# apple/swift-homomorphic-encryption

Hardware: NVIDIA H100
Metric: BFV ct*ct mults/sec at N=8192, 4 coefficient moduli (higher is better)
Workload: dtype u64

## Files before the change

swift-homomorphic-encryption_b200/csrc/behz.cu:

```cuda
#include <cstdlib>

#include "kernels.cuh"
#include "ntt_fast.cuh"

namespace hecuda {

constexpr int kThreads = 128;

static int cols_per_thread() {
    static const int v = [] {
        const char *e = std::getenv("HECUDA_BEHZ_COLS");
        return (e && e[0] == '1') ? 1 : 2;
    }();
    return v;
}

template <int COLS>
struct Cols {
    u64 v[COLS];
};
template <int COLS>
__device__ __forceinline__ Cols<COLS> ldc(const u64 *p) {
    Cols<COLS> r;
    if (COLS == 2) {
        const ulonglong2 t = *reinterpret_cast<const ulonglong2 *>(p);
        r.v[0] = t.x;
        r.v[COLS - 1] = t.y;
    } else {
        r.v[0] = *p;
    }
    return r;
}
template <int COLS>
__device__ __forceinline__ void stc(u64 *p, const u64 (&v)[COLS]) {
    if (COLS == 2) *reinterpret_cast<ulonglong2 *>(p) = make_ulonglong2(v[0], v[COLS - 1]);
    else *p = v[0];
}

template <int L, int COLS, bool H>
__global__ void __launch_bounds__(kThreads) lift_kernel(const u64 *__restrict__ in, int polys_in, u64 *__restrict__ ext,
                                                       int ext_polys, int out_poly_offset,
                                                       const __grid_constant__ LiftConsts c, int n, bool q_rows) {
    const int rows_out = q_rows ? 2 * L + 1 : L + 1, aux0 = q_rows ? L : 0;
    const int coeff = (blockIdx.x * kThreads + threadIdx.x) * COLS;
    if (coeff >= n) return;
    const int64_t poly = (int64_t)blockIdx.z * gridDim.y + blockIdx.y;
    const int64_t item = polys_in == 2 ? (poly >> 1) : poly / polys_in;
    const int pin = (int)(poly - item * polys_in);
    const u64 *src = in + poly * L * n + coeff;
    u64 *dst = ext + ((item * ext_polys + out_poly_offset + pin) * rows_out) * n + coeff;
    u64 z[COLS][L];
    u32 acc_mt[COLS];
#pragma unroll
    for (int k = 0; k < COLS; ++k) acc_mt[k] = 0;
#pragma unroll
    for (int i = 0; i < L; ++i) {
        const Cols<COLS> x = ldc<COLS>(src + (int64_t)i * n);
        if (q_rows) stc<COLS>(dst + (int64_t)i * n, x.v);
#pragma unroll
        for (int k = 0; k < COLS; ++k) {
            z[k][i] = shoup_mul(x.v[k], c.in_w[i], c.in_wp[i], c.q[i]);
            acc_mt[k] += (u32)z[k][i] * c.punct_mt[i];
        }
    }
    u32 r[COLS];
    bool neg[COLS];
#pragma unroll
    for (int k = 0; k < COLS; ++k) {
        r[k] = (acc_mt[k] * c.neg_inv_q_mt) & c.mt_mask;
        neg[k] = r[k] >= c.mt_half;
    }
#pragma unroll
    for (int j = 0; j <= L; ++j) {
        u64 o[COLS];
#pragma unroll
        for (int k = 0; k < COLS; ++k) {
            const u64 rc = neg[k] ? (u64)r[k] + c.neg_off[j] : (u64)r[k];
            u128 acc = (u128)rc * c.qr[j];
#pragma unroll
            for (int i = 0; i < L; ++i) mac128(acc, z[k][i], c.mat[j][i]);
            const u64 red = mont_reduce_c<H>(acc, c.b[j], c.b_ninv[j]);
            o[k] = c.wide_sums ? barrett64(red, c.b[j], c.b_mu1[j]) : csub(red, c.b[j]);
        }
        stc<COLS>(dst + (int64_t)(aux0 + j) * n, o);
    }
}

struct TensorConsts {
    int R;
    u64 p[kMaxRows], ninv[kMaxRows];
    unsigned char h[kMaxRows];
};

template <int COLS, bool H>
__device__ __forceinline__ void tensor_cols(const Cols<COLS> &a0, const Cols<COLS> &a1, const Cols<COLS> &b0,
                                            const Cols<COLS> &b1, u64 p, u64 ninv, u64 (&o0)[COLS], u64 (&o1)[COLS],
                                            u64 (&o2)[COLS]) {
#pragma unroll
    for (int k = 0; k < COLS; ++k) {
        o0[k] = csub(mont_reduce_c<H>((u128)a0.v[k] * b0.v[k], p, ninv), p);
        u128 m = (u128)a0.v[k] * b1.v[k];
        mac128(m, a1.v[k], b0.v[k]);
        o1[k] = csub(mont_reduce_c<H>(m, p, ninv), p);
        o2[k] = csub(mont_reduce_c<H>((u128)a1.v[k] * b1.v[k], p, ninv), p);
    }
}

template <int COLS, bool ANY_H>
__global__ void __launch_bounds__(kThreads) tensor_kernel(const u64 *__restrict__ ext, u64 *__restrict__ ten,
                                                         const __grid_constant__ TensorConsts c, int n) {
    const int R = c.R;
    const int row = blockIdx.y;
    const int64_t item = blockIdx.z;
    const int coeff = (blockIdx.x * kThreads + threadIdx.x) * COLS;
    if (coeff >= n) return;
    const u64 p = c.p[row], ninv = c.ninv[row];
    const u64 *e = ext + (item * 4 * R + row) * n + coeff;
    const int64_t ps = (int64_t)R * n;
    const Cols<COLS> a0 = ldc<COLS>(e), a1 = ldc<COLS>(e + ps), b0 = ldc<COLS>(e + 2 * ps), b1 = ldc<COLS>(e + 3 * ps);
    u64 *o = ten + (item * 3 * R + row) * n + coeff;
    u64 o0[COLS], o1[COLS], o2[COLS];
    if (ANY_H && c.h[row]) tensor_cols<COLS, true>(a0, a1, b0, b1, p, ninv, o0, o1, o2);
    else tensor_cols<COLS, false>(a0, a1, b0, b1, p, ninv, o0, o1, o2);
    stc<COLS>(o, o0);
    stc<COLS>(o + ps, o1);
    stc<COLS>(o + 2 * ps, o2);
}

struct TensorSumConsts {
    int R;
    long long max_pairs;
    u64 p[kMaxRows], ninv[kMaxRows], mu1[kMaxRows], mu_hi[kMaxRows], mu_lo[kMaxRows];
};

__global__ void __launch_bounds__(kThreads) tensor_sum_kernel(const u64 *__restrict__ ext, u64 *__restrict__ ten,
                                                             const __grid_constant__ TensorSumConsts c, int n,
                                                             long long pairs) {
    const int R = c.R;
    const int row = blockIdx.y;
    const int64_t group = blockIdx.z;
    const int coeff = (blockIdx.x * kThreads + threadIdx.x) * 2;
    if (coeff >= n) return;
    const u64 p = c.p[row], ninv = c.ninv[row];
    const int64_t ps = (int64_t)R * n;
    const u64 *e = ext + (group * pairs * 4 * R + row) * n + coeff;
    u128 a0[2] = {0, 0}, a1[2] = {0, 0}, a2[2] = {0, 0};
    long long since = 0;
    for (long long k = 0; k < pairs; ++k, e += 4 * ps) {
        const Cols<2> l0 = ldc<2>(e), l1 = ldc<2>(e + ps), r0 = ldc<2>(e + 2 * ps), r1 = ldc<2>(e + 3 * ps);
#pragma unroll
        for (int j = 0; j < 2; ++j) {
            mac128(a0[j], l0.v[j], r0.v[j]);
            mac128(a1[j], l0.v[j], r1.v[j]);
            mac128(a1[j], l1.v[j], r0.v[j]);
            mac128(a2[j], l1.v[j], r1.v[j]);
        }
        if (++since >= c.max_pairs) {
            since = 0;
#pragma unroll
            for (int j = 0; j < 2; ++j) {
                u128w w0 = {(u64)a0[j], (u64)(a0[j] >> 64)}, w1 = {(u64)a1[j], (u64)(a1[j] >> 64)},
                      w2 = {(u64)a2[j], (u64)(a2[j] >> 64)};
                a0[j] = barrett128(w0, p, c.mu_hi[row], c.mu_lo[row]);
                a1[j] = barrett128(w1, p, c.mu_hi[row], c.mu_lo[row]);
                a2[j] = barrett128(w2, p, c.mu_hi[row], c.mu_lo[row]);
            }
        }
    }
    u64 *o = ten + (group * 3 * R + row) * n + coeff;
    u64 o0[2], o1[2], o2[2];
    const u64 mu1 = c.mu1[row];
#pragma unroll
    for (int j = 0; j < 2; ++j) {
        o0[j] = barrett64(mont_reduce(a0[j], p, ninv), p, mu1);
        o1[j] = barrett64(mont_reduce(a1[j], p, ninv), p, mu1);
        o2[j] = barrett64(mont_reduce(a2[j], p, ninv), p, mu1);
    }
    stc<2>(o, o0);
    stc<2>(o + ps, o1);
    stc<2>(o + 2 * ps, o2);
}

template <int L, int COLS, bool H>
__global__ void __launch_bounds__(kThreads) floor_kernel(const u64 *__restrict__ in, u64 *__restrict__ out,
                                                        const __grid_constant__ FloorConsts c, int n) {
    constexpr int R = 2 * L + 1;
    const int coeff = (blockIdx.x * kThreads + threadIdx.x) * COLS;
    if (coeff >= n) return;
    const int64_t poly = (int64_t)blockIdx.z * gridDim.y + blockIdx.y;
    const u64 *src = in + poly * R * n + coeff;
    u64 *dst = out + poly * L * n + coeff;
    u64 y[COLS][L];
#pragma unroll
    for (int i = 0; i < L; ++i) {
        const Cols<COLS> x = ldc<COLS>(src + (int64_t)i * n);
#pragma unroll
        for (int k = 0; k < COLS; ++k) y[k][i] = shoup_mul(x.v[k], c.inq_w[i], c.inq_wp[i], c.q[i]);
    }
    u64 f[COLS][L + 1];
#pragma unroll
    for (int j = 0; j <= L; ++j) {
        const Cols<COLS> xb = ldc<COLS>(src + (int64_t)(L + j) * n);
#pragma unroll
        for (int k = 0; k < COLS; ++k) {
            u128 acc = (u128)xb.v[k] * c.fq[j];
#pragma unroll
            for (int i = 0; i < L; ++i) mac128(acc, y[k][i], c.fmat[j][i]);
            f[k][j] = mont_reduce_c<H>(acc, c.b[j], c.b_ninv[j]);
        }
    }
    const u64 msk = c.b[L];
    u64 outv[L][COLS];
#pragma unroll
    for (int k = 0; k < COLS; ++k) {
        u64 w[L];
        u128 acc = (u128)f[k][L] * c.a_msk;
#pragma unroll
        for (int i = 0; i < L; ++i) {
            w[i] = shoup_mul(f[k][i], c.inb_w[i], c.inb_wp[i], c.b[i]);
            mac128(acc, w[i], c.amat[i]);
        }
        u64 alpha = mont_reduce_c<H>(acc, msk, c.b_ninv[L]);
        alpha = c.wide_sums ? barrett64(alpha, msk, c.msk_mu1) : csub(csub(csub(alpha, 4 * msk), 2 * msk), msk);
        const bool exceeds = alpha > (msk >> 1);
        const u64 alpha_c = exceeds ? msk - alpha : alpha;
#pragma unroll
        for (int i = 0; i < L; ++i) {
            u128 o = (u128)alpha_c * (exceeds ? c.b_mod_q[i] : c.neg_b_mod_q[i]);
#pragma unroll
            for (int kk = 0; kk < L; ++kk) mac128(o, w[kk], c.omat[i][kk]);
            outv[i][k] = csub(csub(mont_reduce(o, c.q[i], c.q_ninv[i]), 2 * c.q[i]), c.q[i]);
        }
    }
#pragma unroll
    for (int i = 0; i < L; ++i) stc<COLS>(dst + (int64_t)i * n, outv[i]);
}

__global__ void __launch_bounds__(kThreads) lift_generic_kernel(const u64 *__restrict__ in, int polys_in, u64 *__restrict__ ext,
                                                               int ext_polys, int out_poly_offset,
                                                               const __grid_constant__ LiftConsts c, int n, bool q_rows) {
    const int L = c.L, rows_out = q_rows ? 2 * L + 1 : L + 1, aux0 = q_rows ? L : 0;
    const int coeff = blockIdx.x * kThreads + threadIdx.x;
    if (coeff >= n) return;
    const int64_t poly = (int64_t)blockIdx.z * gridDim.y + blockIdx.y;
    const int64_t item = poly / polys_in;
    const int pin = (int)(poly - item * polys_in);
    const u64 *src = in + poly * L * n + coeff;
    u64 *dst = ext + ((item * ext_polys + out_poly_offset + pin) * rows_out) * n + coeff;
    u64 z[kMaxL];
    u32 acc_mt = 0;
    for (int i = 0; i < L; ++i) {
        const u64 x = src[(int64_t)i * n];
        if (q_rows) dst[(int64_t)i * n] = x;
        z[i] = shoup_mul(x, c.in_w[i], c.in_wp[i], c.q[i]);
        acc_mt += (u32)z[i] * c.punct_mt[i];
    }
    const u32 r = (acc_mt * c.neg_inv_q_mt) & c.mt_mask;
    const bool neg = r >= c.mt_half;
    for (int j = 0; j <= L; ++j) {
        const u64 rc = neg ? (u64)r + c.neg_off[j] : (u64)r;
        u128 acc = (u128)rc * c.qr[j];
        for (int i = 0; i < L; ++i) mac128(acc, z[i], c.mat[j][i]);
        const u64 red = mont_reduce(acc, c.b[j], c.b_ninv[j]);
        dst[(int64_t)(aux0 + j) * n] = c.wide_sums ? barrett64(red, c.b[j], c.b_mu1[j]) : csub(red, c.b[j]);
    }
}

__global__ void __launch_bounds__(kThreads) floor_generic_kernel(const u64 *__restrict__ in, u64 *__restrict__ out,
                                                                const __grid_constant__ FloorConsts c, int n) {
    const int L = c.L, R = 2 * L + 1;
    const int coeff = blockIdx.x * kThreads + threadIdx.x;
    if (coeff >= n) return;
    const int64_t poly = (int64_t)blockIdx.z * gridDim.y + blockIdx.y;
    const u64 *src = in + poly * R * n + coeff;
    u64 *dst = out + poly * L * n + coeff;
    u64 y[kMaxL], f[kMaxL + 1], w[kMaxL];
    for (int i = 0; i < L; ++i) y[i] = shoup_mul(src[(int64_t)i * n], c.inq_w[i], c.inq_wp[i], c.q[i]);
    for (int j = 0; j <= L; ++j) {
        u128 acc = (u128)src[(int64_t)(L + j) * n] * c.fq[j];
        for (int i = 0; i < L; ++i) mac128(acc, y[i], c.fmat[j][i]);
        f[j] = mont_reduce(acc, c.b[j], c.b_ninv[j]);
    }
    const u64 msk = c.b[L];
    u128 acc = (u128)f[L] * c.a_msk;
    for (int i = 0; i < L; ++i) {
        w[i] = shoup_mul(f[i], c.inb_w[i], c.inb_wp[i], c.b[i]);
        mac128(acc, w[i], c.amat[i]);
    }
    u64 alpha = mont_reduce(acc, msk, c.b_ninv[L]);
    alpha = c.wide_sums ? barrett64(alpha, msk, c.msk_mu1) : csub(csub(csub(alpha, 4 * msk), 2 * msk), msk);
    const bool exceeds = alpha > (msk >> 1);
    const u64 alpha_c = exceeds ? msk - alpha : alpha;
    for (int i = 0; i < L; ++i) {
        u128 o = (u128)alpha_c * (exceeds ? c.b_mod_q[i] : c.neg_b_mod_q[i]);
        for (int kk = 0; kk < L; ++kk) mac128(o, w[kk], c.omat[i][kk]);
        dst[(int64_t)i * n] = barrett64(mont_reduce(o, c.q[i], c.q_ninv[i]), c.q[i], c.q_mu1[i]);
    }
}

#define HE_DISPATCH_L(L_, CALL)                                                                                       \
    switch (L_) {                                                                                                     \
        case 1: { constexpr int LL = 1; CALL; } break;                                                                \
        case 2: { constexpr int LL = 2; CALL; } break;                                                                \
        case 3: { constexpr int LL = 3; CALL; } break;                                                                \
        case 4: { constexpr int LL = 4; CALL; } break;                                                                \
        case 5: { constexpr int LL = 5; CALL; } break;                                                                \
        case 6: { constexpr int LL = 6; CALL; } break;                                                                \
        case 7: { constexpr int LL = 7; CALL; } break;                                                                \
        case 8: { constexpr int LL = 8; CALL; } break;                                                                \
        case 9: { constexpr int LL = 9; CALL; } break;                                                                \
        case 10: { constexpr int LL = 10; CALL; } break;                                                              \
        case 11: { constexpr int LL = 11; CALL; } break;                                                              \
        case 12: { constexpr int LL = 12; CALL; } break;                                                              \
        case 13: { constexpr int LL = 13; CALL; } break;                                                              \
        case 14: { constexpr int LL = 14; CALL; } break;                                                              \
        case 15: { constexpr int LL = 15; CALL; } break;                                                              \
        case 16: { constexpr int LL = 16; CALL; } break;                                                              \
        default: return cudaErrorInvalidValue;                                                                        \
    }

template <int COLS, bool H>
static cudaError_t launch_lift_kernel(int L, dim3 grid, cudaStream_t stream, const u64 *in, int polys_in, u64 *ext,
                                      int ext_polys, int out_poly_offset, const LiftConsts &consts, int n, bool q_rows) {
    HE_DISPATCH_L(L, (lift_kernel<LL, COLS, H><<<grid, kThreads, 0, stream>>>(in, polys_in, ext, ext_polys, out_poly_offset,
                                                                              consts, n, q_rows)));
    return cudaSuccess;
}
template <int COLS, bool H>
static cudaError_t launch_floor_kernel(int L, dim3 grid, cudaStream_t stream, const u64 *in, u64 *out,
                                       const FloorConsts &consts, int n) {
    HE_DISPATCH_L(L, (floor_kernel<LL, COLS, H><<<grid, kThreads, 0, stream>>>(in, out, consts, n)));
    return cudaSuccess;
}

static inline dim3 poly_grid(int64_t n, int64_t polys, int cols) {
    const unsigned gx = (unsigned)((n / cols + kThreads - 1) / kThreads);
    const int64_t gy = polys < 32768 ? polys : 32768;
    return dim3(gx ? gx : 1, (unsigned)gy, (unsigned)((polys + gy - 1) / gy));
}

cudaError_t launch_lift(const Context &ctx, const u64 *in, int polys_in, u64 *ext, int ext_polys, int out_poly_offset,
                        int64_t items, cudaStream_t stream, bool reference_base, bool q_rows) {
    const LiftConsts &consts = reference_base ? ctx.lift : ctx.lift_mul;
    int64_t polys = items * polys_in;
    if (polys == 0) return cudaSuccess;
    const int64_t pstride_in = (int64_t)ctx.L * ctx.n;
    while (polys > 0) {
        int64_t slab = polys >= 32768 ? (polys / 32768) * 32768 : polys;
        const int cols = ctx.L > 16 ? 1 : (ctx.n >= 2 ? cols_per_thread() : 1);
        const dim3 grid = poly_grid(ctx.n, slab, cols);
        ++g_kernel_launches;
        if (ctx.L > 16) {
            lift_generic_kernel<<<grid, kThreads, 0, stream>>>(in, polys_in, ext, ext_polys, out_poly_offset, consts, (int)ctx.n, q_rows);
        } else {
            auto launch = cols == 2 ? (consts.h_primes ? launch_lift_kernel<2, true> : launch_lift_kernel<2, false>)
                                    : (consts.h_primes ? launch_lift_kernel<1, true> : launch_lift_kernel<1, false>);
            const cudaError_t e = launch(ctx.L, grid, stream, in, polys_in, ext, ext_polys, out_poly_offset, consts, (int)ctx.n, q_rows);
            if (e != cudaSuccess) return e;
        }
        in += slab * pstride_in;
        ext += (slab / polys_in) * (int64_t)ext_polys * (q_rows ? 2 * ctx.L + 1 : ctx.L + 1) * ctx.n;
        polys -= slab;
    }
    return cudaGetLastError();
}

cudaError_t launch_tensor(const Context &ctx, const u64 *ext, u64 *ten, int64_t items, cudaStream_t stream,
                          bool reference_base) {
    if (items == 0) return cudaSuccess;
    TensorConsts tc;
    tc.R = 2 * ctx.L + 1;
    const NttRowMap map = reference_base ? ctx.map_qbsk() : ctx.map_qaux();
    for (int r = 0; r < tc.R; ++r) {
        tc.p[r] = ctx.slots[map.slot[r]].dev.p;
        tc.ninv[r] = ctx.slots[map.slot[r]].dev.ninv;
        tc.h[r] = fast::class_of_modulus(tc.p[r], ctx.slots[map.slot[r]].dev.bits) == fast::kNarrowH ? 1 : 0;
    }
    const int cols = ctx.n >= 2 ? cols_per_thread() : 1;
    bool any_h = false;
    for (int r = 0; r < tc.R; ++r) any_h |= tc.h[r] != 0;
    auto k = cols == 2 ? (any_h ? tensor_kernel<2, true> : tensor_kernel<2, false>) : (any_h ? tensor_kernel<1, true> : tensor_kernel<1, false>);
    const unsigned gx = (unsigned)((ctx.n / cols + kThreads - 1) / kThreads);
    for (int64_t done = 0; done < items;) {
        const int64_t chunk = (items - done) > 65535 ? 65535 : (items - done);
        dim3 grid(gx ? gx : 1, (unsigned)tc.R, (unsigned)chunk);
        ++g_kernel_launches;
        k<<<grid, kThreads, 0, stream>>>(ext + done * 4 * tc.R * ctx.n, ten + done * 3 * tc.R * ctx.n, tc, (int)ctx.n);
        done += chunk;
    }
    return cudaGetLastError();
}

cudaError_t launch_tensor_sum(const Context &ctx, const u64 *ext, u64 *ten, int64_t pairs, int64_t groups,
                              cudaStream_t stream, bool reference_base) {
    if (groups == 0) return cudaSuccess;
    if (ctx.n < 2 || pairs < 1) return cudaErrorInvalidValue;
    TensorSumConsts tc;
    tc.R = 2 * ctx.L + 1;
    const NttRowMap map = reference_base ? ctx.map_qbsk() : ctx.map_qaux();
    u64 pmax = 0;
    for (int r = 0; r < tc.R; ++r) {
        const ModSlot &S = ctx.slots[map.slot[r]].dev;
        tc.p[r] = S.p;
        tc.ninv[r] = S.ninv;
        tc.mu1[r] = S.mu1;
        tc.mu_hi[r] = S.mu_hi;
        tc.mu_lo[r] = S.mu_lo;
        pmax = S.p > pmax ? S.p : pmax;
    }
    const u128 per_pair = 2 * (u128)pmax * pmax;
    const u128 cap = (((u128)1) << 127) / per_pair;
    tc.max_pairs = cap < 1 ? 1 : (cap > (u128)0x7fffffffLL ? 0x7fffffffLL : (long long)cap);
    const unsigned gx = (unsigned)((ctx.n / 2 + kThreads - 1) / kThreads);
    for (int64_t done = 0; done < groups;) {
        const int64_t chunk = (groups - done) > 65535 ? 65535 : (groups - done);
        dim3 grid(gx ? gx : 1, (unsigned)tc.R, (unsigned)chunk);
        ++g_kernel_launches;
        tensor_sum_kernel<<<grid, kThreads, 0, stream>>>(ext + done * pairs * 4 * tc.R * ctx.n, ten + done * 3 * tc.R * ctx.n,
                                                         tc, (int)ctx.n, pairs);
        done += chunk;
    }
    return cudaGetLastError();
}

cudaError_t launch_floor(const Context &ctx, const u64 *in, u64 *out, int64_t polys, cudaStream_t stream,
                         bool reference_base) {
    if (polys == 0) return cudaSuccess;
    const FloorConsts &consts = reference_base ? ctx.floor : ctx.floor_mul;
    const int R = 2 * ctx.L + 1;
    while (polys > 0) {
        int64_t slab = polys >= 32768 ? (polys / 32768) * 32768 : polys;
        const int cols = ctx.L > 16 ? 1 : (ctx.n >= 2 ? cols_per_thread() : 1);
        const dim3 grid = poly_grid(ctx.n, slab, cols);
        ++g_kernel_launches;
        if (ctx.L > 16) {
            floor_generic_kernel<<<grid, kThreads, 0, stream>>>(in, out, consts, (int)ctx.n);
        } else {
            auto launch = cols == 2 ? (consts.h_primes ? launch_floor_kernel<2, true> : launch_floor_kernel<2, false>)
                                    : (consts.h_primes ? launch_floor_kernel<1, true> : launch_floor_kernel<1, false>);
            const cudaError_t e = launch(ctx.L, grid, stream, in, out, consts, (int)ctx.n);
            if (e != cudaSuccess) return e;
        }
        in += slab * (int64_t)R * ctx.n;
        out += slab * (int64_t)ctx.L * ctx.n;
        polys -= slab;
    }
    return cudaGetLastError();
}

}
```

swift-homomorphic-encryption_b200/csrc/capi.cu:

```cuda
#include "../../include/hecuda.h"

#include <cuda_runtime.h>
#include <sched.h>
#include <sys/syscall.h>
#include <unistd.h>

#include <algorithm>
#include <cctype>
#include <cstdio>
#include <cstdlib>
#include <cstring>
#include <map>
#include <memory>
#include <mutex>
#include <new>
#include <string>
#include <vector>

#include "capi_internal.hpp"

namespace hecuda {
std::atomic<unsigned long long> g_kernel_launches{0};
}

using namespace hecuda;

namespace hecuda {
namespace api {

static thread_local std::string tl_error;

int32_t fail(int32_t code, const std::string &msg) {
    tl_error = msg;
    return code;
}
int32_t cuda_fail(cudaError_t e, const char *what) {
    return fail(HECUDA_ERR_CUDA, std::string(what) + ": " + cudaGetErrorString(e));
}
const char *last_error_cstr() { return tl_error.c_str(); }

}
}

using namespace hecuda::api;

namespace hecuda {
namespace api {

cudaError_t wait_stream(cudaStream_t s) {
    static const bool blocking = [] {
        const char *env = std::getenv("HECUDA_BLOCKING_SYNC");
        return !(env && env[0] == '0');
    }();
    if (!blocking) return cudaStreamSynchronize(s);
    thread_local cudaEvent_t event = nullptr;
    thread_local int event_device = -1;
    int device = 0;
    cudaError_t e = cudaGetDevice(&device);
    if (e != cudaSuccess) return e;
    if (!event || event_device != device) {
        if ((e = cudaEventCreateWithFlags(&event, cudaEventBlockingSync | cudaEventDisableTiming)) != cudaSuccess) return e;
        event_device = device;
    }
    if ((e = cudaEventRecord(event, s)) != cudaSuccess) return e;
    return cudaEventSynchronize(event);
}

int32_t check_ctx(const hecuda_context *h) {
    if (!h || !h->ctx) return fail(HECUDA_ERR_INVALID_ARGUMENT, "invalidContext: null context");
    int dev = -1;
    if (cudaGetDevice(&dev) != cudaSuccess) return fail(HECUDA_ERR_NO_DEVICE, "no CUDA device available");
    if (dev != h->ctx->device) {
        cudaError_t e = cudaSetDevice(h->ctx->device);
        if (e != cudaSuccess) return cuda_fail(e, "cudaSetDevice");
    }
    return HECUDA_OK;
}

bool make_map(const Context &c, int32_t base, int32_t rows, NttRowMap &map, std::string &err) {
    switch (base) {
        case HECUDA_BASE_Q:
            if (rows < 1 || rows > c.L) { err = "invalidPolyContext: row_count must be in [1, L] for BASE_Q"; return false; }
            map = c.map_q(rows);
            return true;
        case HECUDA_BASE_Q_BSK:
            if (rows != 2 * c.L + 1) { err = "invalidPolyContext: BASE_Q_BSK needs 2L+1 rows"; return false; }
            map = c.map_qbsk();
            return true;
        case HECUDA_BASE_Q_AUX:
            if (rows != 2 * c.L + 1) { err = "invalidPolyContext: BASE_Q_AUX needs 2L+1 rows"; return false; }
            map = c.map_qaux();
            return true;
        case HECUDA_BASE_KEYSWITCH:
            if (!c.has_ks) { err = "invalidPolyContext: these parameters have no key-switching modulus"; return false; }
            if (rows < 2 || rows > c.L + 1) { err = "invalidPolyContext: BASE_KEYSWITCH needs 2..L+1 rows"; return false; }
            map = c.map_ks(rows - 1);
            return true;
        default:
            err = "invalidPolyContext: unknown base";
            return false;
    }
}


size_t multiply_scratch_words(const Context &c) { return (size_t)7 * (2 * c.L + 1) * c.n; }
size_t relinearize_scratch_words(const Context &c, int l) { return (size_t)((l + 1) * l + 2 * (l + 1)) * c.n; }

cudaError_t multiply_chunk(const Context &c, u64 *scratch, const u64 *lhs, const u64 *rhs, u64 *out, int64_t items,
                           cudaStream_t s) {
    const int R = 2 * c.L + 1;
    const size_t poly_words = (size_t)R * c.n;
    cudaError_t e;
    u64 *ext = scratch, *ten = scratch + 4 * poly_words * items;
    const NttRowMap map = c.map_qaux();
    if (ntt_forward_tensor_supported(c)) {
        if ((e = launch_lift(c, lhs, 2, ext, 4, 0, items, s, false, false)) != cudaSuccess) return e;
        if ((e = launch_lift(c, rhs, 2, ext, 4, 2, items, s, false, false)) != cudaSuccess) return e;
        if ((e = launch_ntt_forward_tensor(c, map, lhs, rhs, ext, ten, items, s)) != cudaSuccess) return e;
        if ((e = launch_ntt_inverse(c, map, ten, ten, items * 3 * R, kScaleTMont, s)) != cudaSuccess) return e;
        return launch_floor(c, ten, out, items * 3, s);
    }
    if ((e = launch_lift(c, lhs, 2, ext, 4, 0, items, s)) != cudaSuccess) return e;
    if ((e = launch_lift(c, rhs, 2, ext, 4, 2, items, s)) != cudaSuccess) return e;
    if ((e = launch_ntt_forward(c, map, ext, ext, items * 4 * R, s)) != cudaSuccess) return e;
    if ((e = launch_tensor(c, ext, ten, items, s)) != cudaSuccess) return e;
    if ((e = launch_ntt_inverse(c, map, ten, ten, items * 3 * R, kScaleTMont, s)) != cudaSuccess) return e;
    return launch_floor(c, ten, out, items * 3, s);
}

cudaError_t keyswitch_chunk(const Context &c, u64 *scratch, const u64 *key, const u64 *target, int64_t target_stride,
                            int l, const u64 *base, int64_t base_stride, int base_mask, u64 *out, int64_t items,
                            cudaStream_t s) {
    const size_t dig_words = (size_t)(l + 1) * l * c.n;
    cudaError_t e;
    u64 *dig = scratch, *prod = scratch + dig_words * items;
    if ((e = launch_ntt_forward(c, c.map_ks_digits(l, target_stride), target, dig, items * (l + 1) * l, s)) != cudaSuccess)
        return e;
    if ((e = launch_ks_mac(c, dig, key, l, prod, items, s)) != cudaSuccess) return e;
    if ((e = launch_ntt_inverse(c, c.map_ks(l), prod, prod, items * 2 * (l + 1), kScaleMont, s)) != cudaSuccess) return e;
    return launch_ks_finish(c, prod, base, base_stride, base_mask, l, out, items, s);
}

cudaError_t relinearize_chunk(const Context &c, u64 *scratch, const u64 *key, const u64 *ct3, int l, u64 *out,
                              int64_t items, cudaStream_t s) {
    const int64_t ct_stride = (int64_t)3 * l * c.n;
    return keyswitch_chunk(c, scratch, key, ct3 + (int64_t)2 * l * c.n, ct_stride, l, ct3, ct_stride, 3, out, items, s);
}

size_t galois_scratch_words(const Context &c, int l) { return relinearize_scratch_words(c, l) + (size_t)l * c.n; }
cudaError_t apply_galois_chunk(const Context &c, u64 *scratch, const u64 *key, const u64 *ct, int l, unsigned element,
                               u64 *out, int64_t items, cudaStream_t s) {
    const int64_t poly = (int64_t)l * c.n, ct_stride = 2 * poly;
    u64 *perm1 = scratch;
    u64 *ks_scratch = scratch + poly * items;
    const NttRowMap map = c.map_q(l);
    cudaError_t e;
    if ((e = launch_galois_coeff(c, map, element, ct, ct_stride, out, ct_stride, items, s)) != cudaSuccess) return e;
    if ((e = launch_galois_coeff(c, map, element, ct + poly, ct_stride, perm1, poly, items, s)) != cudaSuccess) return e;
    return keyswitch_chunk(c, ks_scratch, key, perm1, poly, l, out, ct_stride, 1, out, items, s);
}

cudaError_t inner_product_chunk(const Context &c, u64 *scratch, const u64 *lhs, const u64 *rhs, int64_t pairs,
                                       u64 *out, int64_t groups, cudaStream_t s) {
    const int R = 2 * c.L + 1;
    const size_t poly_words = (size_t)R * c.n;
    const int64_t items = groups * pairs;
    u64 *ext = scratch, *ten = scratch + 4 * poly_words * items;
    const NttRowMap map = c.map_qaux();
    cudaError_t e;
    if ((e = launch_lift(c, lhs, 2, ext, 4, 0, items, s)) != cudaSuccess) return e;
    if ((e = launch_lift(c, rhs, 2, ext, 4, 2, items, s)) != cudaSuccess) return e;
    if ((e = launch_ntt_forward(c, map, ext, ext, items * 4 * R, s)) != cudaSuccess) return e;
    if ((e = launch_tensor_sum(c, ext, ten, pairs, groups, s)) != cudaSuccess) return e;
    if ((e = launch_ntt_inverse(c, map, ten, ten, groups * 3 * R, kScaleTMont, s)) != cudaSuccess) return e;
    return launch_floor(c, ten, out, groups * 3, s);
}
size_t inner_product_scratch_words(const Context &c, int64_t pairs) {
    return (size_t)(4 * pairs + 3) * (2 * c.L + 1) * c.n;
}

}
}

namespace {

thread_local bool tl_io32 = false;
struct Io32Scope {
    Io32Scope() { tl_io32 = true; }
    ~Io32Scope() { tl_io32 = false; }
};

struct HostIo {
    const u64 *src;
    size_t words_per_item;
};
template <class Body>
int32_t host_pipeline(const hecuda_context *h, int64_t batch, int64_t chunk_hint, size_t scratch_words_per_item,
                      const std::vector<HostIo> &inputs, u64 *host_out, size_t out_words_per_item, Body body) {
    if (batch == 0) return HECUDA_OK;
    static const int depth = [] {
        const char *env = std::getenv("HECUDA_PIPELINE_DEPTH");
        const int d = env ? std::atoi(env) : 3;
        return d < 1 ? 1 : (d > 8 ? 8 : d);
    }();
    static const int64_t min_stages = [] {
        const char *env = std::getenv("HECUDA_PIPELINE_STAGES");
        const long long v = env ? std::atoll(env) : 16;
        return (int64_t)(v < 1 ? 1 : v);
    }();
    std::vector<std::unique_ptr<WsGuard>> guards;
    std::vector<Workspace *> ws;
    for (int i = 0; i < depth; ++i) {
        guards.emplace_back(new WsGuard(h));
        if (!guards.back()->w) return fail(HECUDA_ERR_CUDA, "could not create a CUDA stream / workspace");
        ws.push_back(guards.back()->w);
    }
    int64_t chunk = std::max<int64_t>(1, std::min<int64_t>(chunk_hint, batch));
    if (batch >= 64) chunk = std::min<int64_t>(chunk, std::max<int64_t>(16, (batch + min_stages - 1) / min_stages));
    struct DrainOnExit {
        std::vector<Workspace *> &ws;
        ~DrainOnExit() {
            for (Workspace *w : ws) wait_stream(w->stream);
        }
    } drain{ws};
    int k = 0;
    for (int64_t done = 0; done < batch; done += chunk, ++k) {
        Workspace &w = *ws[k % depth];
        const int64_t items = std::min<int64_t>(chunk, batch - done);
        size_t in_words = 0;
        for (const HostIo &io : inputs) in_words += io.words_per_item * (size_t)items;
        const bool io32 = tl_io32;
        const size_t out_words = out_words_per_item * (size_t)items;
        CK(w.reserve(0, scratch_words_per_item * (size_t)items));
        CK(w.reserve(4, in_words));
        CK(w.reserve(5, out_words));
        if (io32) {
            CK(w.reserve(6, in_words / 2 + inputs.size() * 2 + 2));
            CK(w.reserve(7, out_words / 2 + 2));
        }
        std::vector<const u64 *> d_in;
        size_t off = 0, off32 = 0;
        for (const HostIo &io : inputs) {
            const size_t words = io.words_per_item * (size_t)items;
            if (io32) {
                u32 *raw = reinterpret_cast<u32 *>(w.buf[6]) + off32;
                CK(cudaMemcpyAsync(raw, reinterpret_cast<const u32 *>(io.src) + io.words_per_item * (size_t)done,
                                   words * sizeof(u32), cudaMemcpyHostToDevice, w.stream));
                CK(launch_widen(raw, w.buf[4] + off, (int64_t)words, w.stream));
                off32 += (words + 3) & ~(size_t)3;
            } else {
                CK(cudaMemcpyAsync(w.buf[4] + off, io.src + io.words_per_item * (size_t)done, words * sizeof(u64),
                                   cudaMemcpyHostToDevice, w.stream));
            }
            d_in.push_back(w.buf[4] + off);
            off += words;
        }
        cudaError_t e = body(w, d_in, w.buf[5], items);
        if (e != cudaSuccess) return cuda_fail(e, "kernel launch");
        if (io32) {
            CK(launch_narrow(w.buf[5], reinterpret_cast<u32 *>(w.buf[7]), (int64_t)out_words, w.stream));
            CK(cudaMemcpyAsync(reinterpret_cast<u32 *>(host_out) + out_words_per_item * (size_t)done, w.buf[7],
                               out_words * sizeof(u32), cudaMemcpyDeviceToHost, w.stream));
        } else {
            CK(cudaMemcpyAsync(host_out + out_words_per_item * (size_t)done, w.buf[5], out_words * sizeof(u64),
                               cudaMemcpyDeviceToHost, w.stream));
        }
    }
    for (Workspace *w : ws) CK(wait_stream(w->stream));
    return HECUDA_OK;
}

}


extern "C" {

int32_t hecuda_version(void) { return 100; }
const char *hecuda_last_error(void) { return last_error_cstr(); }

int32_t hecuda_device_count(int32_t *count) {
    if (!count) return fail(HECUDA_ERR_INVALID_ARGUMENT, "null count");
    int n = 0;
    cudaError_t e = cudaGetDeviceCount(&n);
    if (e != cudaSuccess) {
        *count = 0;
        return fail(HECUDA_ERR_NO_DEVICE, std::string("no CUDA device: ") + cudaGetErrorString(e));
    }
    *count = n;
    return HECUDA_OK;
}
int32_t hecuda_set_device(int32_t device) {
    CK(cudaSetDevice(device));
    return HECUDA_OK;
}

int32_t hecuda_bind_host_to_device(int32_t device, int32_t *numa_node, int32_t *cpu_count) {
    if (numa_node) *numa_node = -1;
    if (cpu_count) *cpu_count = 0;
    char bus[32] = {0};
    CK(cudaDeviceGetPCIBusId(bus, sizeof(bus), device));
    for (char *c = bus; *c; ++c) *c = (char)std::tolower((unsigned char)*c);
    const std::string dir = std::string("/sys/bus/pci/devices/") + bus + "/";
    int node = -1;
    if (FILE *f = std::fopen((dir + "numa_node").c_str(), "r")) {
        if (std::fscanf(f, "%d", &node) != 1) node = -1;
        std::fclose(f);
    }
    char list[4096] = {0};
    if (FILE *f = std::fopen((dir + "local_cpulist").c_str(), "r")) {
        if (!std::fgets(list, sizeof(list), f)) list[0] = 0;
        std::fclose(f);
    }
    cpu_set_t current, want;
    CPU_ZERO(&want);
    if (sched_getaffinity(0, sizeof(current), &current) != 0) return HECUDA_OK;
    int picked = 0;
    char *save = nullptr;
    for (char *tok = strtok_r(list, ",\n", &save); tok; tok = strtok_r(nullptr, ",\n", &save)) {
        int lo = 0, hi = 0;
        const int fields = std::sscanf(tok, "%d-%d", &lo, &hi);
        if (fields < 1) continue;
        if (fields == 1) hi = lo;
        for (int c = lo; c <= hi && c < CPU_SETSIZE; ++c)
            if (CPU_ISSET(c, &current)) {
                CPU_SET(c, &want);
                ++picked;
            }
    }
    if (picked > 0) sched_setaffinity(0, sizeof(want), &want);
    if (node >= 0 && node < 64) {
        unsigned long mask = 1ul << node;
        syscall(SYS_set_mempolicy, 1 , &mask, sizeof(mask) * 8);
    }
    if (numa_node) *numa_node = node;
    if (cpu_count) *cpu_count = picked;
    return HECUDA_OK;
}

int32_t hecuda_host_alloc(void **ptr, uint64_t bytes) {
    if (!ptr) return fail(HECUDA_ERR_INVALID_ARGUMENT, "null ptr");
    CK(cudaHostAlloc(ptr, bytes, cudaHostAllocDefault));
    return HECUDA_OK;
}
int32_t hecuda_host_free(void *ptr) {
    CK(cudaFreeHost(ptr));
    return HECUDA_OK;
}
int32_t hecuda_host_register(void *ptr, uint64_t bytes) {
    CK(cudaHostRegister(ptr, bytes, cudaHostRegisterDefault));
    return HECUDA_OK;
}
int32_t hecuda_host_unregister(void *ptr) {
    CK(cudaHostUnregister(ptr));
    return HECUDA_OK;
}

static int32_t context_create(int64_t poly_degree, const uint64_t *coefficient_moduli, int32_t moduli_count,
                              uint64_t plaintext_modulus, int word_bits, hecuda_context **out);
int32_t hecuda_context_create(int64_t poly_degree, const uint64_t *coefficient_moduli, int32_t moduli_count,
                              uint64_t plaintext_modulus, hecuda_context **out) {
    return context_create(poly_degree, coefficient_moduli, moduli_count, plaintext_modulus, 64, out);
}
int32_t hecuda_context_create_u32(int64_t poly_degree, const uint32_t *coefficient_moduli, int32_t moduli_count,
                                  uint32_t plaintext_modulus, hecuda_context **out) {
    if (!coefficient_moduli || moduli_count < 0) return fail(HECUDA_ERR_INVALID_ARGUMENT, "null argument");
    std::vector<uint64_t> wide(coefficient_moduli, coefficient_moduli + moduli_count);
    return context_create(poly_degree, wide.data(), moduli_count, plaintext_modulus, 32, out);
}
int32_t hecuda_context_word_bits(const hecuda_context *h, int32_t *bits) {
    if (!h || !bits) return fail(HECUDA_ERR_INVALID_ARGUMENT, "null argument");
    *bits = h->ctx->word_bits;
    return HECUDA_OK;
}
static int32_t context_create(int64_t poly_degree, const uint64_t *coefficient_moduli, int32_t moduli_count,
                              uint64_t plaintext_modulus, int word_bits, hecuda_context **out) {
    if (!out || !coefficient_moduli) return fail(HECUDA_ERR_INVALID_ARGUMENT, "null argument");
    *out = nullptr;
    int ndev = 0;
    if (cudaGetDeviceCount(&ndev) != cudaSuccess || ndev == 0)
        return fail(HECUDA_ERR_NO_DEVICE, "no CUDA device: libhecuda has no CPU fallback");
    std::string err;
    Context *c = Context::create(poly_degree, (const u64 *)coefficient_moduli, moduli_count, plaintext_modulus, err, word_bits);
    if (!c) {
        const bool unsupported = err.rfind("unsupported", 0) == 0;
        return fail(unsupported ? HECUDA_ERR_UNSUPPORTED : HECUDA_ERR_INVALID_ARGUMENT, err);
    }
    hecuda_context *h = new (std::nothrow) hecuda_context();
    if (!h) {
        delete c;
        return fail(HECUDA_ERR_CUDA, "out of host memory");
    }
    h->ctx = c;
    {
        cudaMemPool_t pool;
        if (cudaDeviceGetDefaultMemPool(&pool, c->device) == cudaSuccess) {
            unsigned long long threshold = ~0ull;
            cudaMemPoolSetAttribute(pool, cudaMemPoolAttrReleaseThreshold, &threshold);
        }
    }
    const size_t per_item = (size_t)7 * (2 * c->L + 1) * c->n * sizeof(u64);
    int64_t chunk = (int64_t)((size_t)2048 * 1024 * 1024 / per_item);
    if (const char *env = std::getenv("HECUDA_CHUNK")) chunk = std::atoll(env);
    h->chunk = std::max<int64_t>(1, std::min<int64_t>(chunk, 4096));
    context_registered(h, true);
    *out = h;
    return HECUDA_OK;
}

int32_t hecuda_context_destroy(hecuda_context *h) {
    if (!h) return HECUDA_OK;
    if (h->ctx) cudaSetDevice(h->ctx->device);
    cudaDeviceSynchronize();
    pir_graphs_purge(h, nullptr);
    context_registered(h, false);
    for (Workspace *w : h->free_ws) {
        w->release();
        delete w;
    }
    delete h->ctx;
    delete h;
    return HECUDA_OK;
}

int32_t hecuda_context_ciphertext_moduli_count(const hecuda_context *h, int32_t *count) {
    if (!h || !count) return fail(HECUDA_ERR_INVALID_ARGUMENT, "null argument");
    *count = h->ctx->L;
    return HECUDA_OK;
}
int32_t hecuda_context_bsk_moduli(const hecuda_context *h, uint64_t *out, int32_t capacity, int32_t *count) {
    if (!h || !count) return fail(HECUDA_ERR_INVALID_ARGUMENT, "null argument");
    *count = (int32_t)h->ctx->bsk.size();
    if (out) {
        if (capacity < *count) return fail(HECUDA_ERR_INVALID_ARGUMENT, "capacity too small");
        std::memcpy(out, h->ctx->bsk.data(), sizeof(u64) * h->ctx->bsk.size());
    }
    return HECUDA_OK;
}
int32_t hecuda_context_aux_moduli(const hecuda_context *h, uint64_t *out, int32_t capacity, int32_t *count) {
    if (!h || !count) return fail(HECUDA_ERR_INVALID_ARGUMENT, "null argument");
    *count = (int32_t)h->ctx->aux.size();
    if (out) {
        if (capacity < *count) return fail(HECUDA_ERR_INVALID_ARGUMENT, "capacity too small");
        std::memcpy(out, h->ctx->aux.data(), sizeof(u64) * h->ctx->aux.size());
    }
    return HECUDA_OK;
}
int32_t hecuda_context_root_tables(const hecuda_context *h, uint64_t modulus, uint64_t *roots, uint64_t *inverse_roots) {
    if (!h) return fail(HECUDA_ERR_INVALID_ARGUMENT, "null context");
    const int s = h->ctx->find_slot(modulus);
    if (s < 0) return fail(HECUDA_ERR_INVALID_ARGUMENT, "invalidNttModulus: modulus is not part of this context");
    if (roots) std::memcpy(roots, h->ctx->slots[s].roots.data(), sizeof(u64) * h->ctx->n);
    if (inverse_roots) std::memcpy(inverse_roots, h->ctx->slots[s].inv_roots.data(), sizeof(u64) * h->ctx->n);
    return HECUDA_OK;
}


static int32_t ntt_device(const hecuda_context *h, int32_t base, uint64_t *data, int32_t rows, int64_t polys,
                          void *stream, bool inverse) {
    int32_t rc = check_ctx(h);
    if (rc) return rc;
    if (polys < 0 || (!data && polys)) return fail(HECUDA_ERR_INVALID_ARGUMENT, "invalid data / poly_count");
    NttRowMap map;
    std::string err;
    if (!make_map(*h->ctx, base, rows, map, err)) return fail(HECUDA_ERR_INVALID_ARGUMENT, err);
    cudaError_t e = inverse ? launch_ntt_inverse(*h->ctx, map, (u64 *)data, (u64 *)data, polys * rows, kScalePlain,
                                                 (cudaStream_t)stream)
                            : launch_ntt_forward(*h->ctx, map, (u64 *)data, (u64 *)data, polys * rows,
                                                 (cudaStream_t)stream);
    if (e != cudaSuccess) return cuda_fail(e, "ntt launch");
    return HECUDA_OK;
}
int32_t hecuda_ntt_forward_device(const hecuda_context *h, int32_t base, uint64_t *data, int32_t rows, int64_t polys,
                                  void *stream) {
    return ntt_device(h, base, data, rows, polys, stream, false);
}
int32_t hecuda_ntt_inverse_device(const hecuda_context *h, int32_t base, uint64_t *data, int32_t rows, int64_t polys,
                                  void *stream) {
    return ntt_device(h, base, data, rows, polys, stream, true);
}

static int32_t ntt_host(const hecuda_context *h, const NttRowMap &map, uint64_t *data, size_t words_per_item,
                        int64_t items, int64_t rows_per_item, bool inverse) {
    const Context &c = *h->ctx;
    std::vector<HostIo> in = {{(const u64 *)data, words_per_item}};
    const int64_t chunk = std::max<int64_t>(1, (int64_t)((size_t)4 * 1024 * 1024 / std::max<size_t>(1, words_per_item)));
    return host_pipeline(h, items, chunk, 0, in, (u64 *)data, words_per_item,
                         [&](Workspace &w, const std::vector<const u64 *> &d_in, u64 *d_out, int64_t n_items) {
                             return inverse ? launch_ntt_inverse(c, map, d_in[0], d_out, n_items * rows_per_item, kScalePlain,
                                                                 w.stream)
                                            : launch_ntt_forward(c, map, d_in[0], d_out, n_items * rows_per_item,
                                                                 w.stream);
                         });
}
int32_t hecuda_ntt_forward(const hecuda_context *h, int32_t base, uint64_t *data, int32_t rows, int64_t polys) {
    int32_t rc = check_ctx(h);
    if (rc) return rc;
    if (polys < 0 || (!data && polys)) return fail(HECUDA_ERR_INVALID_ARGUMENT, "invalid data / poly_count");
    NttRowMap map;
    std::string err;
    if (!make_map(*h->ctx, base, rows, map, err)) return fail(HECUDA_ERR_INVALID_ARGUMENT, err);
    return ntt_host(h, map, data, (size_t)rows * h->ctx->n, polys, rows, false);
}
int32_t hecuda_ntt_inverse(const hecuda_context *h, int32_t base, uint64_t *data, int32_t rows, int64_t polys) {
    int32_t rc = check_ctx(h);
    if (rc) return rc;
    if (polys < 0 || (!data && polys)) return fail(HECUDA_ERR_INVALID_ARGUMENT, "invalid data / poly_count");
    NttRowMap map;
    std::string err;
    if (!make_map(*h->ctx, base, rows, map, err)) return fail(HECUDA_ERR_INVALID_ARGUMENT, err);
    return ntt_host(h, map, data, (size_t)rows * h->ctx->n, polys, rows, true);
}
int32_t hecuda_rnstool_lift_q_to_qbsk(const hecuda_context *h, const uint64_t *polys, uint64_t *out, int64_t count) {
    int32_t rc = check_ctx(h);
    if (rc) return rc;
    if (count < 0 || ((!polys || !out) && count)) return fail(HECUDA_ERR_INVALID_ARGUMENT, "invalid buffers / poly_count");
    const Context &c = *h->ctx;
    const size_t in_words = (size_t)c.L * c.n, out_words = (size_t)(2 * c.L + 1) * c.n;
    std::vector<HostIo> in = {{(const u64 *)polys, in_words}};
    return host_pipeline(h, count, std::max<int64_t>(1, (int64_t)((size_t)4 * 1024 * 1024 / out_words)), 0, in, (u64 *)out, out_words,
                         [&](Workspace &w, const std::vector<const u64 *> &d_in, u64 *d_out, int64_t n_items) {
                             return launch_lift(c, d_in[0], 1, d_out, 1, 0, n_items, w.stream, true);
                         });
}
int32_t hecuda_rnstool_floor_qbsk_to_q(const hecuda_context *h, const uint64_t *polys, uint64_t *out, int64_t count) {
    int32_t rc = check_ctx(h);
    if (rc) return rc;
    if (count < 0 || ((!polys || !out) && count)) return fail(HECUDA_ERR_INVALID_ARGUMENT, "invalid buffers / poly_count");
    const Context &c = *h->ctx;
    const size_t in_words = (size_t)(2 * c.L + 1) * c.n, out_words = (size_t)c.L * c.n;
    std::vector<HostIo> in = {{(const u64 *)polys, in_words}};
    return host_pipeline(h, count, std::max<int64_t>(1, (int64_t)((size_t)4 * 1024 * 1024 / in_words)), 0, in, (u64 *)out, out_words,
                         [&](Workspace &w, const std::vector<const u64 *> &d_in, u64 *d_out, int64_t n_items) {
                             return launch_floor(c, d_in[0], d_out, n_items, w.stream, true);
                         });
}

static int32_t ntt_rows_host(const hecuda_context *h, uint64_t modulus, uint64_t *data, int64_t rows, bool inverse) {
    int32_t rc = check_ctx(h);
    if (rc) return rc;
    if (rows < 0 || (!data && rows)) return fail(HECUDA_ERR_INVALID_ARGUMENT, "invalid data / row_count");
    const int s = h->ctx->find_slot(modulus);
    if (s < 0) return fail(HECUDA_ERR_INVALID_ARGUMENT, "invalidPolyContext: modulus is not part of this context");
    return ntt_host(h, h->ctx->map_single(s), data, (size_t)h->ctx->n, rows, 1, inverse);
}
int32_t hecuda_ntt_forward_rows(const hecuda_context *h, uint64_t modulus, uint64_t *data, int64_t rows) {
    return ntt_rows_host(h, modulus, data, rows, false);
}
int32_t hecuda_ntt_inverse_rows(const hecuda_context *h, uint64_t modulus, uint64_t *data, int64_t rows) {
    return ntt_rows_host(h, modulus, data, rows, true);
}


int32_t hecuda_bfv_multiply_device(const hecuda_context *h, const uint64_t *lhs, const uint64_t *rhs, uint64_t *out,
                                   int64_t batch, void *stream) {
    int32_t rc = check_ctx(h);
    if (rc) return rc;
    if (batch < 0 || (batch && (!lhs || !rhs || !out))) return fail(HECUDA_ERR_INVALID_ARGUMENT, "invalidCiphertext: null buffer");
    if (batch == 0) return HECUDA_OK;
    const Context &c = *h->ctx;
    const size_t in_words = (size_t)2 * c.L * c.n, out_words = (size_t)3 * c.L * c.n;
    const int64_t chunk = std::max<int64_t>(1, std::min<int64_t>(h->chunk, batch));
    cudaStream_t s = (cudaStream_t)stream;
    u64 *scratch = nullptr;
    CK(cudaMallocAsync(&scratch, multiply_scratch_words(c) * (size_t)chunk * sizeof(u64), s));
    for (int64_t done = 0; done < batch; done += chunk) {
        const int64_t items = std::min<int64_t>(chunk, batch - done);
        cudaError_t e = multiply_chunk(c, scratch, (const u64 *)lhs + in_words * done, (const u64 *)rhs + in_words * done,
                                       (u64 *)out + out_words * done, items, s);
        if (e != cudaSuccess) {
            cudaFreeAsync(scratch, s);
            return cuda_fail(e, "multiply");
        }
    }
    CK(cudaFreeAsync(scratch, s));
    return HECUDA_OK;
}

int32_t hecuda_bfv_multiply(const hecuda_context *h, const uint64_t *lhs, const uint64_t *rhs, uint64_t *out,
                            int64_t batch) {
    int32_t rc = check_ctx(h);
    if (rc) return rc;
    if (batch < 0 || (batch && (!lhs || !rhs || !out))) return fail(HECUDA_ERR_INVALID_ARGUMENT, "invalidCiphertext: null buffer");
    const Context &c = *h->ctx;
    const size_t in_words = (size_t)2 * c.L * c.n, out_words = (size_t)3 * c.L * c.n;
    std::vector<HostIo> in = {{(const u64 *)lhs, in_words}, {(const u64 *)rhs, in_words}};
    return host_pipeline(h, batch, h->chunk, multiply_scratch_words(c), in, (u64 *)out, out_words,
                         [&](Workspace &w, const std::vector<const u64 *> &d_in, u64 *d_out, int64_t items) {
                             return multiply_chunk(c, w.buf[0], d_in[0], d_in[1], d_out, items, w.stream);
                         });
}


int32_t hecuda_evk_create_empty(const hecuda_context *h, hecuda_evk **out) {
    int32_t rc = check_ctx(h);
    if (rc) return rc;
    if (!out) return fail(HECUDA_ERR_INVALID_ARGUMENT, "null argument");
    const Context &c = *h->ctx;
    if (!c.has_ks)
        return fail(HECUDA_ERR_UNSUPPORTED, "unsupportedHeOperation: a single coefficient modulus leaves no key-switching modulus");
    hecuda_evk *k = new (std::nothrow) hecuda_evk();
    if (!k) return fail(HECUDA_ERR_CUDA, "out of host memory");
    k->owner = h;
    k->words = (size_t)c.L * 2 * (c.L + 1) * c.n;
    cudaError_t e = cudaMalloc(&k->d_relin, k->words * sizeof(u64));
    if (e != cudaSuccess) {
        delete k;
        return cuda_fail(e, "cudaMalloc(evk)");
    }
    *out = k;
    return HECUDA_OK;
}
int32_t hecuda_evk_create(const hecuda_context *h, const uint64_t *relin_key, hecuda_evk **out) {
    if (!relin_key) return fail(HECUDA_ERR_MISSING_KEY, "missingRelinearizationKey");
    int32_t rc = hecuda_evk_create_empty(h, out);
    if (rc) return rc;
    cudaError_t e = upload((*out)->d_relin, relin_key, (*out)->words * sizeof(u64));
    if (e != cudaSuccess) {
        hecuda_evk_destroy(*out);
        *out = nullptr;
        return cuda_fail(e, "cudaMemcpy(evk)");
    }
    (*out)->loaded = true;
    return HECUDA_OK;
}
int32_t hecuda_evk_destroy(hecuda_evk *k) {
    if (!k) return HECUDA_OK;
    if (k->owner) pir_graphs_purge(const_cast<hecuda_context *>(k->owner), k);
    if (k->d_relin) cudaFree(k->d_relin);
    for (auto &kv : k->galois) cudaFree(kv.second);
    for (hecuda::u64 *p : k->retired) cudaFree(p);
    delete k;
    return HECUDA_OK;
}
int32_t hecuda_evk_device_buffer(hecuda_evk *k, void **device_ptr, uint64_t *bytes) {
    if (!k || !device_ptr || !bytes) return fail(HECUDA_ERR_INVALID_ARGUMENT, "null argument");
    *device_ptr = k->d_relin;
    *bytes = k->words * sizeof(u64);
    k->loaded = true;
    ++k->version;
    return HECUDA_OK;
}


static int32_t check_relin(const hecuda_context *h, const hecuda_evk *k, const uint64_t *ct3, int32_t l, uint64_t *out,
                           int64_t batch) {
    int32_t rc = check_ctx(h);
    if (rc) return rc;
    if (!k || !k->loaded) return fail(HECUDA_ERR_MISSING_KEY, "missingRelinearizationKey");
    if (k->owner != h) return fail(HECUDA_ERR_INVALID_ARGUMENT, "invalidContext: evaluation key belongs to another context");
    if (l < 1 || l > h->ctx->L) return fail(HECUDA_ERR_INVALID_ARGUMENT, "invalidCiphertext: moduli_count out of range");
    if (batch < 0 || (batch && (!ct3 || !out))) return fail(HECUDA_ERR_INVALID_ARGUMENT, "invalidCiphertext: null buffer");
    return HECUDA_OK;
}

int32_t hecuda_bfv_relinearize_device(const hecuda_context *h, const hecuda_evk *k, const uint64_t *ct3, int32_t l,
                                      uint64_t *out, int64_t batch, void *stream) {
    int32_t rc = check_relin(h, k, ct3, l, out, batch);
    if (rc) return rc;
    if (batch == 0) return HECUDA_OK;
    const Context &c = *h->ctx;
    const size_t in_words = (size_t)3 * l * c.n, out_words = (size_t)2 * l * c.n;
    const int64_t chunk = std::max<int64_t>(1, std::min<int64_t>(h->chunk, batch));
    cudaStream_t s = (cudaStream_t)stream;
    u64 *scratch = nullptr;
    CK(cudaMallocAsync(&scratch, relinearize_scratch_words(c, l) * (size_t)chunk * sizeof(u64), s));
    for (int64_t done = 0; done < batch; done += chunk) {
        const int64_t items = std::min<int64_t>(chunk, batch - done);
        cudaError_t e = relinearize_chunk(c, scratch, k->d_relin, (const u64 *)ct3 + in_words * done, l,
                                          (u64 *)out + out_words * done, items, s);
        if (e != cudaSuccess) {
            cudaFreeAsync(scratch, s);
            return cuda_fail(e, "relinearize");
        }
    }
    CK(cudaFreeAsync(scratch, s));
    return HECUDA_OK;
}

int32_t hecuda_bfv_relinearize(const hecuda_context *h, const hecuda_evk *k, const uint64_t *ct3, int32_t l,
                               uint64_t *out, int64_t batch) {
    int32_t rc = check_relin(h, k, ct3, l, out, batch);
    if (rc) return rc;
    const Context &c = *h->ctx;
    std::vector<HostIo> in = {{(const u64 *)ct3, (size_t)3 * l * c.n}};
    return host_pipeline(h, batch, h->chunk, relinearize_scratch_words(c, l), in, (u64 *)out, (size_t)2 * l * c.n,
                         [&](Workspace &w, const std::vector<const u64 *> &d_in, u64 *d_out, int64_t items) {
                             return relinearize_chunk(c, w.buf[0], k->d_relin, d_in[0], l, d_out, items, w.stream);
                         });
}

static int32_t check_ms(const hecuda_context *h, const uint64_t *ct, int32_t polys, int32_t l, uint64_t *out,
                        int64_t batch) {
    int32_t rc = check_ctx(h);
    if (rc) return rc;
    if (polys < 1) return fail(HECUDA_ERR_INVALID_ARGUMENT, "invalidCiphertext: poly_count");
    if (l < 2 || l > h->ctx->L)
        return fail(HECUDA_ERR_INVALID_ARGUMENT, "invalidPolyContext: modSwitchDown needs a next context (2 <= moduli_count <= L)");
    if (batch < 0 || (batch && (!ct || !out))) return fail(HECUDA_ERR_INVALID_ARGUMENT, "invalidCiphertext: null buffer");
    return HECUDA_OK;
}

int32_t hecuda_bfv_mod_switch_down_device(const hecuda_context *h, const uint64_t *ct, int32_t polys, int32_t l,
                                          uint64_t *out, int64_t batch, void *stream) {
    int32_t rc = check_ms(h, ct, polys, l, out, batch);
    if (rc) return rc;
    cudaError_t e = launch_mod_switch(*h->ctx, (const u64 *)ct, l, (u64 *)out, batch * polys, (cudaStream_t)stream);
    if (e != cudaSuccess) return cuda_fail(e, "mod_switch");
    return HECUDA_OK;
}

int32_t hecuda_bfv_mod_switch_down(const hecuda_context *h, const uint64_t *ct, int32_t polys, int32_t l, uint64_t *out,
                                   int64_t batch) {
    int32_t rc = check_ms(h, ct, polys, l, out, batch);
    if (rc) return rc;
    const Context &c = *h->ctx;
    std::vector<HostIo> in = {{(const u64 *)ct, (size_t)polys * l * c.n}};
    const int64_t chunk = std::max<int64_t>(1, (int64_t)((size_t)4 * 1024 * 1024 / ((size_t)polys * l * c.n)));
    return host_pipeline(h, batch, chunk, 0, in, (u64 *)out, (size_t)polys * (l - 1) * c.n,
                         [&](Workspace &w, const std::vector<const u64 *> &d_in, u64 *d_out, int64_t items) {
                             return launch_mod_switch(c, d_in[0], l, d_out, items * polys, w.stream);
                         });
}


int32_t hecuda_bfv_relinearize_mod_switch_down(const hecuda_context *h, const hecuda_evk *k, const uint64_t *ct3, int32_t l,
                                               uint64_t *out, int64_t batch) {
    int32_t rc = check_relin(h, k, ct3, l, out, batch);
    if (rc) return rc;
    if (l < 2) return fail(HECUDA_ERR_INVALID_ARGUMENT, "invalidPolyContext: modSwitchDown needs a next context (moduli_count >= 2)");
    const Context &c = *h->ctx;
    const size_t relin_words = (size_t)2 * l * c.n;
    std::vector<HostIo> in = {{(const u64 *)ct3, (size_t)3 * l * c.n}};
    return host_pipeline(h, batch, h->chunk, relinearize_scratch_words(c, l) + relin_words, in, (u64 *)out, (size_t)2 * (l - 1) * c.n,
                         [&](Workspace &w, const std::vector<const u64 *> &d_in, u64 *d_out, int64_t items) {
                             u64 *relin = w.buf[0] + relinearize_scratch_words(c, l) * (size_t)items;
                             cudaError_t e = relinearize_chunk(c, w.buf[0], k->d_relin, d_in[0], l, relin, items, w.stream);
                             if (e != cudaSuccess) return e;
                             return launch_mod_switch(c, relin, l, d_out, items * 2, w.stream);
                         });
}

static size_t mul_relin_scratch_words(const Context &c) {
    return multiply_scratch_words(c) + (size_t)3 * c.L * c.n + relinearize_scratch_words(c, c.L) + (size_t)2 * c.L * c.n;
}
static cudaError_t mul_relin_chunk(const Context &c, u64 *scratch, const u64 *key, const u64 *lhs, const u64 *rhs, bool mod_switch,
                                   u64 *out, int64_t items, cudaStream_t s) {
    u64 *mul_scratch = scratch;
    u64 *prod = mul_scratch + multiply_scratch_words(c) * (size_t)items;
    u64 *ks_scratch = prod + (size_t)3 * c.L * c.n * items;
    u64 *relin = ks_scratch + relinearize_scratch_words(c, c.L) * (size_t)items;
    cudaError_t e;
    if ((e = multiply_chunk(c, mul_scratch, lhs, rhs, prod, items, s)) != cudaSuccess) return e;
    if ((e = relinearize_chunk(c, ks_scratch, key, prod, c.L, mod_switch ? relin : out, items, s)) != cudaSuccess) return e;
    if (mod_switch) return launch_mod_switch(c, relin, c.L, out, items * 2, s);
    return cudaSuccess;
}
static int32_t check_mul_relin(const hecuda_context *h, const hecuda_evk *k, const void *lhs, const void *rhs, const void *out,
                               int32_t mod_switch, int64_t batch) {
    int32_t rc = check_ctx(h);
    if (rc) return rc;
    if (!k || !k->loaded) return fail(HECUDA_ERR_MISSING_KEY, "missingRelinearizationKey");
    if (k->owner != h) return fail(HECUDA_ERR_INVALID_ARGUMENT, "invalidContext: evaluation key belongs to another context");
    if (mod_switch && h->ctx->L < 2)
        return fail(HECUDA_ERR_INVALID_ARGUMENT, "invalidPolyContext: modSwitchDown needs a next context (L >= 2)");
    if (batch < 0 || (batch && (!lhs || !rhs || !out))) return fail(HECUDA_ERR_INVALID_ARGUMENT, "invalidCiphertext: null buffer");
    return HECUDA_OK;
}
int32_t hecuda_bfv_multiply_relinearize_device(const hecuda_context *h, const hecuda_evk *k, const uint64_t *lhs,
                                               const uint64_t *rhs, int32_t mod_switch, uint64_t *out, int64_t batch,
                                               void *stream) {
    int32_t rc = check_mul_relin(h, k, lhs, rhs, out, mod_switch, batch);
    if (rc || batch == 0) return rc;
    const Context &c = *h->ctx;
    const size_t in_words = (size_t)2 * c.L * c.n, out_words = (size_t)2 * (c.L - (mod_switch ? 1 : 0)) * c.n;
    const int64_t chunk = std::max<int64_t>(1, std::min<int64_t>(h->chunk / 2, batch));
    cudaStream_t s = (cudaStream_t)stream;
    u64 *scratch = nullptr;
    CK(cudaMallocAsync(&scratch, mul_relin_scratch_words(c) * (size_t)chunk * sizeof(u64), s));
    for (int64_t done = 0; done < batch; done += chunk) {
        const int64_t items = std::min<int64_t>(chunk, batch - done);
        cudaError_t e = mul_relin_chunk(c, scratch, k->d_relin, (const u64 *)lhs + in_words * done, (const u64 *)rhs + in_words * done,
                                        mod_switch != 0, (u64 *)out + out_words * done, items, s);
        if (e != cudaSuccess) {
            cudaFreeAsync(scratch, s);
            return cuda_fail(e, "multiply_relinearize");
        }
    }
    CK(cudaFreeAsync(scratch, s));
    return HECUDA_OK;
}
int32_t hecuda_bfv_multiply_relinearize(const hecuda_context *h, const hecuda_evk *k, const uint64_t *lhs, const uint64_t *rhs,
                                        int32_t mod_switch, uint64_t *out, int64_t batch) {
    int32_t rc = check_mul_relin(h, k, lhs, rhs, out, mod_switch, batch);
    if (rc) return rc;
    const Context &c = *h->ctx;
    const size_t in_words = (size_t)2 * c.L * c.n, out_words = (size_t)2 * (c.L - (mod_switch ? 1 : 0)) * c.n;
    std::vector<HostIo> in = {{(const u64 *)lhs, in_words}, {(const u64 *)rhs, in_words}};
    return host_pipeline(h, batch, std::max<int64_t>(1, h->chunk / 2), mul_relin_scratch_words(c), in, (u64 *)out, out_words,
                         [&](Workspace &w, const std::vector<const u64 *> &d_in, u64 *d_out, int64_t items) {
                             return mul_relin_chunk(c, w.buf[0], k->d_relin, d_in[0], d_in[1], mod_switch != 0, d_out, items,
                                                    w.stream);
                         });
}


static bool valid_galois_element(int64_t element, int64_t n) {
    return (element & 1) && element > 1 && element < 2 * n;
}

int32_t hecuda_evk_set_galois_key(hecuda_evk *k, uint32_t element, const uint64_t *key) {
    if (!k || !key) return fail(HECUDA_ERR_INVALID_ARGUMENT, "null argument");
    int32_t rc = check_ctx(k->owner);
    if (rc) return rc;
    if (!valid_galois_element(element, k->owner->ctx->n)) return fail(HECUDA_ERR_INVALID_ARGUMENT, "invalid Galois element");
    u64 *d = nullptr;
    CK(cudaMalloc(&d, k->words * sizeof(u64)));
    cudaError_t e = upload(d, key, k->words * sizeof(u64));
    if (e != cudaSuccess) {
        cudaFree(d);
        return cuda_fail(e, "cudaMemcpy(galois key)");
    }
    std::lock_guard<std::mutex> g(k->mu);
    auto it = k->galois.find(element);
    if (it != k->galois.end()) {
        k->retired.push_back(it->second);
        it->second = d;
    } else {
        k->galois[element] = d;
    }
    ++k->version;
    return HECUDA_OK;
}

int32_t hecuda_evk_galois_device_buffer(hecuda_evk *k, uint32_t element, void **device_ptr, uint64_t *bytes) {
    if (!k || !device_ptr || !bytes) return fail(HECUDA_ERR_INVALID_ARGUMENT, "null argument");
    int32_t rc = check_ctx(k->owner);
    if (rc) return rc;
    if (!valid_galois_element(element, k->owner->ctx->n)) return fail(HECUDA_ERR_INVALID_ARGUMENT, "invalid Galois element");
    std::lock_guard<std::mutex> g(k->mu);
    auto it = k->galois.find(element);
    if (it == k->galois.end()) {
        u64 *d = nullptr;
        CK(cudaMalloc(&d, k->words * sizeof(u64)));
        it = k->galois.emplace(element, d).first;
    }
    *device_ptr = it->second;
    *bytes = k->words * sizeof(u64);
    return HECUDA_OK;
}

static int32_t check_galois(const hecuda_context *h, const hecuda_evk *k, const uint64_t *ct, int32_t l, uint32_t element,
                            uint64_t *out, int64_t batch, const u64 **key) {
    int32_t rc = check_ctx(h);
    if (rc) return rc;
    if (!k) return fail(HECUDA_ERR_MISSING_KEY, "missingGaloisKey");
    if (k->owner != h) return fail(HECUDA_ERR_INVALID_ARGUMENT, "invalidContext: evaluation key belongs to another context");
    if (!valid_galois_element(element, h->ctx->n)) return fail(HECUDA_ERR_INVALID_ARGUMENT, "invalid Galois element");
    if (l < 1 || l > h->ctx->L) return fail(HECUDA_ERR_INVALID_ARGUMENT, "invalidCiphertext: moduli_count out of range");
    if (batch < 0 || (batch && (!ct || !out))) return fail(HECUDA_ERR_INVALID_ARGUMENT, "invalidCiphertext: null buffer");
    hecuda_evk *km = const_cast<hecuda_evk *>(k);
    std::lock_guard<std::mutex> g(km->mu);
    auto it = km->galois.find(element);
    if (it == km->galois.end()) return fail(HECUDA_ERR_MISSING_KEY, "missingGaloisElement: " + std::to_string(element));
    *key = it->second;
    return HECUDA_OK;
}

int32_t hecuda_bfv_apply_galois_device(const hecuda_context *h, const hecuda_evk *k, const uint64_t *ct, int32_t l,
                                       uint32_t element, uint64_t *out, int64_t batch, void *stream) {
    const u64 *key = nullptr;
    int32_t rc = check_galois(h, k, ct, l, element, out, batch, &key);
    if (rc) return rc;
    if (batch == 0) return HECUDA_OK;
    const Context &c = *h->ctx;
    const size_t words = (size_t)2 * l * c.n;
    const int64_t chunk = std::max<int64_t>(1, std::min<int64_t>(h->chunk, batch));
    cudaStream_t s = (cudaStream_t)stream;
    u64 *scratch = nullptr;
    CK(cudaMallocAsync(&scratch, galois_scratch_words(c, l) * (size_t)chunk * sizeof(u64), s));
    for (int64_t done = 0; done < batch; done += chunk) {
        const int64_t items = std::min<int64_t>(chunk, batch - done);
        cudaError_t e = apply_galois_chunk(c, scratch, key, (const u64 *)ct + words * done, l, element,
                                           (u64 *)out + words * done, items, s);
        if (e != cudaSuccess) {
            cudaFreeAsync(scratch, s);
            return cuda_fail(e, "applyGalois");
        }
    }
    CK(cudaFreeAsync(scratch, s));
    return HECUDA_OK;
}

int32_t hecuda_bfv_apply_galois(const hecuda_context *h, const hecuda_evk *k, const uint64_t *ct, int32_t l,
                                uint32_t element, uint64_t *out, int64_t batch) {
    const u64 *key = nullptr;
    int32_t rc = check_galois(h, k, ct, l, element, out, batch, &key);
    if (rc) return rc;
    const Context &c = *h->ctx;
    std::vector<HostIo> in = {{(const u64 *)ct, (size_t)2 * l * c.n}};
    return host_pipeline(h, batch, h->chunk, galois_scratch_words(c, l), in, (u64 *)out, (size_t)2 * l * c.n,
                         [&](Workspace &w, const std::vector<const u64 *> &d_in, u64 *d_out, int64_t items) {
                             return apply_galois_chunk(c, w.buf[0], key, d_in[0], l, element, d_out, items, w.stream);
                         });
}

int32_t hecuda_poly_apply_galois(const hecuda_context *h, int32_t base, int32_t eval_format, const uint64_t *in,
                                 uint64_t *out, int32_t rows, int64_t polys, uint32_t element) {
    int32_t rc = check_ctx(h);
    if (rc) return rc;
    if (polys < 0 || (polys && (!in || !out))) return fail(HECUDA_ERR_INVALID_ARGUMENT, "invalid data / poly_count");
    if (!valid_galois_element(element, h->ctx->n)) return fail(HECUDA_ERR_INVALID_ARGUMENT, "invalid Galois element");
    NttRowMap map;
    std::string err;
    if (!make_map(*h->ctx, base, rows, map, err)) return fail(HECUDA_ERR_INVALID_ARGUMENT, err);
    const Context &c = *h->ctx;
    const size_t words = (size_t)rows * c.n;
    std::vector<HostIo> hin = {{(const u64 *)in, words}};
    const int64_t chunk = std::max<int64_t>(1, (int64_t)((size_t)4 * 1024 * 1024 / words));
    return host_pipeline(h, polys, chunk, 0, hin, (u64 *)out, words,
                         [&](Workspace &w, const std::vector<const u64 *> &d_in, u64 *d_out, int64_t items) {
                             return eval_format ? launch_galois_eval(c, rows, element, d_in[0], d_out, items, w.stream)
                                                : launch_galois_coeff(c, map, element, d_in[0], (int64_t)words, d_out,
                                                                      (int64_t)words, items, w.stream);
                         });
}


static int32_t check_ip(const hecuda_context *h, const uint64_t *cts, int32_t polys, int32_t l, int64_t terms,
                        const uint64_t *pts, uint64_t *out, int64_t out_count) {
    int32_t rc = check_ctx(h);
    if (rc) return rc;
    if (polys < 1 || polys > 3) return fail(HECUDA_ERR_INVALID_ARGUMENT, "invalidCiphertext: poly_count must be 1..3");
    if (l < 1 || l > h->ctx->L) return fail(HECUDA_ERR_INVALID_ARGUMENT, "invalidCiphertext: moduli_count out of range");
    if (terms < 1) return fail(HECUDA_ERR_INVALID_ARGUMENT, "Empty ciphertexts");
    if (out_count < 0 || (out_count && (!cts || !pts || !out))) return fail(HECUDA_ERR_INVALID_ARGUMENT, "null buffer");
    if (h->ctx->n < 2) return fail(HECUDA_ERR_UNSUPPORTED, "degree too small");
    return HECUDA_OK;
}

int32_t hecuda_bfv_inner_product_plaintexts_device(const hecuda_context *h, const uint64_t *cts, int32_t polys,
                                                   int32_t l, int64_t terms, const uint64_t *pts,
                                                   const uint8_t *present, uint64_t *out, int64_t out_count,
                                                   void *stream) {
    int32_t rc = check_ip(h, cts, polys, l, terms, pts, out, out_count);
    if (rc) return rc;
    cudaError_t e = launch_inner_product_plain(*h->ctx, (const u64 *)cts, polys, l, terms, (const u64 *)pts, present,
                                               (u64 *)out, out_count, (cudaStream_t)stream);
    if (e != cudaSuccess) return cuda_fail(e, "inner_product");
    return HECUDA_OK;
}

int32_t hecuda_bfv_inner_product_plaintexts(const hecuda_context *h, const uint64_t *cts, int32_t polys, int32_t l,
                                            int64_t terms, const uint64_t *pts, const uint8_t *present, uint64_t *out,
                                            int64_t out_count) {
    int32_t rc = check_ip(h, cts, polys, l, terms, pts, out, out_count);
    if (rc) return rc;
    if (out_count == 0) return HECUDA_OK;
    const Context &c = *h->ctx;
    const size_t ct_words = (size_t)terms * polys * l * c.n;
    u64 *d_cts = nullptr;
    unsigned char *d_present = nullptr;
    CK(cudaMalloc(&d_cts, ct_words * sizeof(u64)));
    cudaError_t e = upload(d_cts, cts, ct_words * sizeof(u64));
    if (e == cudaSuccess && present) {
        e = cudaMalloc(&d_present, (size_t)out_count * terms);
        if (e == cudaSuccess) e = upload(d_present, present, (size_t)out_count * terms);
    }
    if (e != cudaSuccess) {
        cudaFree(d_cts);
        cudaFree(d_present);
        return cuda_fail(e, "inner_product upload");
    }
    const size_t pt_words = (size_t)terms * l * c.n;
    std::vector<HostIo> in = {{(const u64 *)pts, pt_words}};
    const int64_t chunk = std::max<int64_t>(1, (int64_t)((size_t)32 * 1024 * 1024 / pt_words));
    int64_t done_items = 0;
    rc = host_pipeline(h, out_count, chunk, 0, in, (u64 *)out, (size_t)polys * l * c.n,
                       [&](Workspace &w, const std::vector<const u64 *> &d_in, u64 *d_out, int64_t items) {
                           const unsigned char *pr = d_present ? d_present + done_items * terms : nullptr;
                           done_items += items;
                           return launch_inner_product_plain(c, d_cts, polys, l, terms, d_in[0], pr, d_out, items, w.stream);
                       });
    cudaDeviceSynchronize();
    cudaFree(d_cts);
    cudaFree(d_present);
    return rc;
}

int32_t hecuda_plaintext_to_eval_device(const hecuda_context *h, const uint64_t *plain, int32_t l, uint64_t *out,
                                        int64_t count, void *stream) {
    int32_t rc = check_ctx(h);
    if (rc) return rc;
    if (l < 1 || l > h->ctx->L) return fail(HECUDA_ERR_INVALID_ARGUMENT, "invalidPolyContext: moduli_count out of range");
    if (count < 0 || (count && (!plain || !out))) return fail(HECUDA_ERR_INVALID_ARGUMENT, "null buffer");
    cudaError_t e = launch_plaintext_to_eval(*h->ctx, (const u64 *)plain, l, (u64 *)out, count, (cudaStream_t)stream);
    if (e != cudaSuccess) return cuda_fail(e, "plaintext_to_eval");
    return HECUDA_OK;
}

int32_t hecuda_plaintext_to_eval(const hecuda_context *h, const uint64_t *plain, int32_t l, uint64_t *out,
                                 int64_t count) {
    int32_t rc = check_ctx(h);
    if (rc) return rc;
    if (l < 1 || l > h->ctx->L) return fail(HECUDA_ERR_INVALID_ARGUMENT, "invalidPolyContext: moduli_count out of range");
    if (count < 0 || (count && (!plain || !out))) return fail(HECUDA_ERR_INVALID_ARGUMENT, "null buffer");
    const Context &c = *h->ctx;
    std::vector<HostIo> in = {{(const u64 *)plain, (size_t)c.n}};
    const int64_t chunk = std::max<int64_t>(1, (int64_t)((size_t)4 * 1024 * 1024 / ((size_t)l * c.n)));
    return host_pipeline(h, count, chunk, 0, in, (u64 *)out, (size_t)l * c.n,
                         [&](Workspace &w, const std::vector<const u64 *> &d_in, u64 *d_out, int64_t items) {
                             return launch_plaintext_to_eval(c, d_in[0], l, d_out, items, w.stream);
                         });
}


int32_t hecuda_context_supports_simd(const hecuda_context *h, int32_t *supported) {
    if (!h || !h->ctx || !supported) return fail(HECUDA_ERR_INVALID_ARGUMENT, "null argument");
    *supported = h->ctx->simd ? 1 : 0;
    return HECUDA_OK;
}

}

namespace {

int32_t need_simd(const hecuda_context *h) {
    int32_t rc = check_ctx(h);
    if (rc) return rc;
    if (!h->ctx->simd)
        return fail(HECUDA_ERR_UNSUPPORTED, "simdEncodingNotSupported: the plaintext modulus is not a prime = 1 mod 2N");
    return HECUDA_OK;
}

bool host_values_below(const void *p, size_t count, u64 t) {
    if (tl_io32) {
        const uint32_t *v = static_cast<const uint32_t *>(p);
        return std::all_of(v, v + count, [t](uint32_t x) { return x < t; });
    }
    const uint64_t *v = static_cast<const uint64_t *>(p);
    return std::all_of(v, v + count, [t](uint64_t x) { return x < t; });
}

int32_t check_encode(const hecuda_context *h, const void *values, int32_t value_count, int32_t l, const void *out,
                     int64_t count) {
    int32_t rc = need_simd(h);
    if (rc) return rc;
    const Context &c = *h->ctx;
    if (value_count < 0 || value_count > c.n)
        return fail(HECUDA_ERR_INVALID_ARGUMENT, "encodingDataCountExceedsLimit: value_count must be in [0, N]");
    if (l < 0 || l > c.L) return fail(HECUDA_ERR_INVALID_ARGUMENT, "invalidPolyContext: moduli_count must be in [0, L]");
    if (count < 0 || (count && (!out || (value_count && !values)))) return fail(HECUDA_ERR_INVALID_ARGUMENT, "null buffer");
    return HECUDA_OK;
}

int32_t check_decode(const hecuda_context *h, const void *plain, int32_t l, const void *values, int64_t count) {
    int32_t rc = need_simd(h);
    if (rc) return rc;
    if (l < 0 || l > h->ctx->L) return fail(HECUDA_ERR_INVALID_ARGUMENT, "invalidPolyContext: moduli_count must be in [0, L]");
    if (count < 0 || (count && (!plain || !values))) return fail(HECUDA_ERR_INVALID_ARGUMENT, "null buffer");
    return HECUDA_OK;
}

int32_t check_translate(const hecuda_context *h, const void *ct, int32_t polys, int32_t l, const void *pt, int64_t pt_count,
                        int32_t op, const void *out, int64_t batch) {
    int32_t rc = check_ctx(h);
    if (rc) return rc;
    if (polys < 2 || polys > 3) return fail(HECUDA_ERR_INVALID_ARGUMENT, "invalidCiphertext: poly_count must be 2 or 3");
    if (l < 1 || l > h->ctx->L) return fail(HECUDA_ERR_INVALID_ARGUMENT, "invalidCiphertext: moduli_count must be in [1, L]");
    if (op < HECUDA_PLAINTEXT_ADD || op > HECUDA_PLAINTEXT_SUB_FROM) return fail(HECUDA_ERR_INVALID_ARGUMENT, "unknown op");
    if (batch < 0) return fail(HECUDA_ERR_INVALID_ARGUMENT, "invalidCiphertext: negative batch");
    if (pt_count != 1 && pt_count != batch)
        return fail(HECUDA_ERR_INVALID_ARGUMENT, "incompatibleCiphertextAndPlaintext: plaintext_count must be 1 or batch");
    if (batch && (!ct || !pt || !out)) return fail(HECUDA_ERR_INVALID_ARGUMENT, "null buffer");
    return HECUDA_OK;
}

int64_t simd_chunk(const Context &c) { return std::max<int64_t>(1, ((int64_t)1 << 25) / c.n); }

}

extern "C" {

int32_t hecuda_bfv_encode_simd_device(const hecuda_context *h, const uint64_t *values, int32_t value_count,
                                      int32_t moduli_count, uint64_t *out, int64_t count, void *stream) {
    int32_t rc = check_encode(h, values, value_count, moduli_count, out, count);
    if (rc || count == 0) return rc;
    const Context &c = *h->ctx;
    cudaStream_t s = (cudaStream_t)stream;
    const int64_t chunk = std::min<int64_t>(simd_chunk(c), count);
    const size_t scratch_words = simd_scratch_words(c, true, moduli_count) * (size_t)chunk;
    u64 *scratch = nullptr;
    if (scratch_words) CK(cudaMallocAsync(&scratch, scratch_words * sizeof(u64), s));
    const int64_t out_words = (int64_t)(moduli_count ? moduli_count : 1) * c.n;
    cudaError_t e = cudaSuccess;
    for (int64_t done = 0; e == cudaSuccess && done < count; done += chunk)
        e = launch_encode_simd(c, (const u64 *)values + done * value_count, value_count, moduli_count,
                               (u64 *)out + done * out_words, scratch, std::min<int64_t>(chunk, count - done), s);
    if (scratch) cudaFreeAsync(scratch, s);
    return e == cudaSuccess ? HECUDA_OK : cuda_fail(e, "encodeSimd");
}

int32_t hecuda_bfv_encode_simd(const hecuda_context *h, const uint64_t *values, int32_t value_count, int32_t moduli_count,
                               uint64_t *out, int64_t count) {
    int32_t rc = check_encode(h, values, value_count, moduli_count, out, count);
    if (rc) return rc;
    const Context &c = *h->ctx;
    if (!host_values_below(values, (size_t)count * value_count, c.t))
        return fail(HECUDA_ERR_INVALID_ARGUMENT, "encodingDataOutOfBounds: values must be below the plaintext modulus");
    const int l = moduli_count;
    std::vector<HostIo> in;
    if (value_count) in.push_back({(const u64 *)values, (size_t)value_count});
    const size_t out_words = (size_t)(l ? l : 1) * c.n;
    const int64_t chunk = std::max<int64_t>(1, (int64_t)((size_t)4 * 1024 * 1024 / out_words));
    return host_pipeline(h, count, chunk, simd_scratch_words(c, true, l), in, (u64 *)out, out_words,
                         [&](Workspace &w, const std::vector<const u64 *> &d_in, u64 *d_out, int64_t items) {
                             return launch_encode_simd(c, d_in.empty() ? nullptr : d_in[0], value_count, l, d_out, w.buf[0],
                                                       items, w.stream);
                         });
}

int32_t hecuda_bfv_decode_simd_device(const hecuda_context *h, const uint64_t *plaintexts, int32_t moduli_count,
                                      uint64_t *values, int64_t count, void *stream) {
    int32_t rc = check_decode(h, plaintexts, moduli_count, values, count);
    if (rc || count == 0) return rc;
    const Context &c = *h->ctx;
    cudaStream_t s = (cudaStream_t)stream;
    const int64_t chunk = std::min<int64_t>(simd_chunk(c), count);
    u64 *scratch = nullptr;
    CK(cudaMallocAsync(&scratch, simd_scratch_words(c, false, moduli_count) * (size_t)chunk * sizeof(u64), s));
    const int64_t in_words = (int64_t)(moduli_count ? moduli_count : 1) * c.n;
    cudaError_t e = cudaSuccess;
    for (int64_t done = 0; e == cudaSuccess && done < count; done += chunk)
        e = launch_decode_simd(c, (const u64 *)plaintexts + done * in_words, moduli_count, (u64 *)values + done * c.n, scratch,
                               std::min<int64_t>(chunk, count - done), s);
    cudaFreeAsync(scratch, s);
    return e == cudaSuccess ? HECUDA_OK : cuda_fail(e, "decodeSimd");
}

int32_t hecuda_bfv_decode_simd(const hecuda_context *h, const uint64_t *plaintexts, int32_t moduli_count, uint64_t *values,
                               int64_t count) {
    int32_t rc = check_decode(h, plaintexts, moduli_count, values, count);
    if (rc) return rc;
    const Context &c = *h->ctx;
    const int l = moduli_count;
    const size_t in_words = (size_t)(l ? l : 1) * c.n;
    std::vector<HostIo> in = {{(const u64 *)plaintexts, in_words}};
    const int64_t chunk = std::max<int64_t>(1, (int64_t)((size_t)4 * 1024 * 1024 / in_words));
    return host_pipeline(h, count, chunk, simd_scratch_words(c, false, l), in, (u64 *)values, (size_t)c.n,
                         [&](Workspace &w, const std::vector<const u64 *> &d_in, u64 *d_out, int64_t items) {
                             return launch_decode_simd(c, d_in[0], l, d_out, w.buf[0], items, w.stream);
                         });
}

int32_t hecuda_bfv_plaintext_translate_device(const hecuda_context *h, const uint64_t *ct, int32_t poly_count,
                                              int32_t moduli_count, const uint64_t *plaintexts, int64_t plaintext_count,
                                              int32_t op, uint64_t *out, int64_t batch, void *stream) {
    int32_t rc = check_translate(h, ct, poly_count, moduli_count, plaintexts, plaintext_count, op, out, batch);
    if (rc) return rc;
    cudaError_t e = launch_plaintext_translate(*h->ctx, (const u64 *)ct, poly_count, moduli_count, (const u64 *)plaintexts,
                                               plaintext_count == 1, op, (u64 *)out, batch, (cudaStream_t)stream);
    return e == cudaSuccess ? HECUDA_OK : cuda_fail(e, "plaintextTranslate");
}

int32_t hecuda_bfv_plaintext_translate(const hecuda_context *h, const uint64_t *ct, int32_t poly_count, int32_t moduli_count,
                                       const uint64_t *plaintexts, int64_t plaintext_count, int32_t op, uint64_t *out,
                                       int64_t batch) {
    int32_t rc = check_translate(h, ct, poly_count, moduli_count, plaintexts, plaintext_count, op, out, batch);
    if (rc || batch == 0) return rc;
    const Context &c = *h->ctx;
    if (!host_values_below(plaintexts, (size_t)plaintext_count * c.n, c.t))
        return fail(HECUDA_ERR_INVALID_ARGUMENT, "encodingDataOutOfBounds: plaintext coefficients must be below t");
    const bool broadcast = plaintext_count == 1;
    const int l = moduli_count;
    const size_t ct_words = (size_t)poly_count * l * c.n;
    std::vector<HostIo> in = {{(const u64 *)ct, ct_words}};
    u64 *d_pt = nullptr;
    if (broadcast) {
        std::vector<u64> pt(c.n);
        if (tl_io32) std::copy((const uint32_t *)plaintexts, (const uint32_t *)plaintexts + c.n, pt.begin());
        else std::copy(plaintexts, plaintexts + c.n, pt.begin());
        CK(cudaMalloc(&d_pt, sizeof(u64) * (size_t)c.n));
        cudaError_t e = upload(d_pt, pt.data(), sizeof(u64) * (size_t)c.n);
        if (e != cudaSuccess) {
            cudaFree(d_pt);
            return cuda_fail(e, "plaintext upload");
        }
    } else {
        in.push_back({(const u64 *)plaintexts, (size_t)c.n});
    }
    const int64_t chunk = std::max<int64_t>(1, (int64_t)((size_t)4 * 1024 * 1024 / ct_words));
    rc = host_pipeline(h, batch, chunk, 0, in, (u64 *)out, ct_words,
                       [&](Workspace &w, const std::vector<const u64 *> &d_in, u64 *d_out, int64_t items) {
                           return launch_plaintext_translate(c, d_in[0], poly_count, l, broadcast ? d_pt : d_in[1], broadcast,
                                                             op, d_out, items, w.stream);
                       });
    if (d_pt) cudaFree(d_pt);
    return rc;
}


static int32_t check_ipc(const hecuda_context *h, const uint64_t *lhs, const uint64_t *rhs, uint64_t *out, int64_t pairs,
                         int64_t groups) {
    int32_t rc = check_ctx(h);
    if (rc) return rc;
    if (pairs < 1) return fail(HECUDA_ERR_INVALID_ARGUMENT, "Empty ciphertexts");
    if (groups < 0 || (groups && (!lhs || !rhs || !out))) return fail(HECUDA_ERR_INVALID_ARGUMENT, "invalidCiphertext: null buffer");
    if (h->ctx->n < 2) return fail(HECUDA_ERR_UNSUPPORTED, "degree too small");
    return HECUDA_OK;
}

int32_t hecuda_bfv_inner_product_device(const hecuda_context *h, const uint64_t *lhs, const uint64_t *rhs, uint64_t *out,
                                        int64_t pairs, int64_t groups, void *stream) {
    int32_t rc = check_ipc(h, lhs, rhs, out, pairs, groups);
    if (rc) return rc;
    if (groups == 0) return HECUDA_OK;
    const Context &c = *h->ctx;
    const size_t in_words = (size_t)pairs * 2 * c.L * c.n, out_words = (size_t)3 * c.L * c.n;
    const int64_t chunk = std::max<int64_t>(1, std::min<int64_t>(std::max<int64_t>(1, h->chunk / pairs), groups));
    cudaStream_t s = (cudaStream_t)stream;
    u64 *scratch = nullptr;
    CK(cudaMallocAsync(&scratch, inner_product_scratch_words(c, pairs) * (size_t)chunk * sizeof(u64), s));
    for (int64_t done = 0; done < groups; done += chunk) {
        const int64_t g = std::min<int64_t>(chunk, groups - done);
        cudaError_t e = inner_product_chunk(c, scratch, (const u64 *)lhs + in_words * done, (const u64 *)rhs + in_words * done,
                                            pairs, (u64 *)out + out_words * done, g, s);
        if (e != cudaSuccess) {
            cudaFreeAsync(scratch, s);
            return cuda_fail(e, "innerProduct");
        }
    }
    CK(cudaFreeAsync(scratch, s));
    return HECUDA_OK;
}

int32_t hecuda_bfv_inner_product(const hecuda_context *h, const uint64_t *lhs, const uint64_t *rhs, uint64_t *out,
                                 int64_t pairs, int64_t groups) {
    int32_t rc = check_ipc(h, lhs, rhs, out, pairs, groups);
    if (rc) return rc;
    const Context &c = *h->ctx;
    const size_t in_words = (size_t)pairs * 2 * c.L * c.n;
    std::vector<HostIo> in = {{(const u64 *)lhs, in_words}, {(const u64 *)rhs, in_words}};
    const int64_t chunk = std::max<int64_t>(1, h->chunk / pairs);
    return host_pipeline(h, groups, chunk, inner_product_scratch_words(c, pairs), in, (u64 *)out, (size_t)3 * c.L * c.n,
                         [&](Workspace &w, const std::vector<const u64 *> &d_in, u64 *d_out, int64_t g) {
                             return inner_product_chunk(c, w.buf[0], d_in[0], d_in[1], pairs, d_out, g, w.stream);
                         });
}

int32_t hecuda_poly_multiply_power_of_x(const hecuda_context *h, int32_t base, const uint64_t *in, uint64_t *out,
                                        int32_t rows, int64_t polys, int64_t power) {
    int32_t rc = check_ctx(h);
    if (rc) return rc;
    if (polys < 0 || (polys && (!in || !out))) return fail(HECUDA_ERR_INVALID_ARGUMENT, "invalid data / poly_count");
    NttRowMap map;
    std::string err;
    if (!make_map(*h->ctx, base, rows, map, err)) return fail(HECUDA_ERR_INVALID_ARGUMENT, err);
    const Context &c = *h->ctx;
    const size_t words = (size_t)rows * c.n;
    std::vector<HostIo> hin = {{(const u64 *)in, words}};
    const int64_t chunk = std::max<int64_t>(1, (int64_t)((size_t)4 * 1024 * 1024 / words));
    return host_pipeline(h, polys, chunk, 0, hin, (u64 *)out, words,
                         [&](Workspace &w, const std::vector<const u64 *> &d_in, u64 *d_out, int64_t items) {
                             return launch_multiply_power_of_x(c, map, power, d_in[0], d_out, items, w.stream);
                         });
}

uint64_t hecuda_kernel_launch_count(void) { return g_kernel_launches.load(); }


static int32_t need_word32(const hecuda_context *h) {
    if (!h || !h->ctx) return fail(HECUDA_ERR_INVALID_ARGUMENT, "invalidContext: null context");
    if (h->ctx->word_bits != 32) return fail(HECUDA_ERR_INVALID_ARGUMENT, "invalidContext: not a Bfv<UInt32> context (hecuda_context_create_u32)");
    return HECUDA_OK;
}
int32_t hecuda_u32_ntt_forward(const hecuda_context *h, int32_t base, uint32_t *data, int32_t rows, int64_t polys) {
    int32_t rc = need_word32(h);
    if (rc) return rc;
    Io32Scope scope;
    return hecuda_ntt_forward(h, base, reinterpret_cast<uint64_t *>(data), rows, polys);
}
int32_t hecuda_u32_ntt_inverse(const hecuda_context *h, int32_t base, uint32_t *data, int32_t rows, int64_t polys) {
    int32_t rc = need_word32(h);
    if (rc) return rc;
    Io32Scope scope;
    return hecuda_ntt_inverse(h, base, reinterpret_cast<uint64_t *>(data), rows, polys);
}
int32_t hecuda_u32_bfv_multiply(const hecuda_context *h, const uint32_t *lhs, const uint32_t *rhs, uint32_t *out, int64_t batch) {
    int32_t rc = need_word32(h);
    if (rc) return rc;
    Io32Scope scope;
    return hecuda_bfv_multiply(h, reinterpret_cast<const uint64_t *>(lhs), reinterpret_cast<const uint64_t *>(rhs),
                               reinterpret_cast<uint64_t *>(out), batch);
}
int32_t hecuda_u32_evk_create(const hecuda_context *h, const uint32_t *relin_key, hecuda_evk **out) {
    int32_t rc = need_word32(h);
    if (rc) return rc;
    if (!relin_key) return fail(HECUDA_ERR_MISSING_KEY, "missingRelinearizationKey");
    const Context &c = *h->ctx;
    const size_t words = (size_t)c.L * 2 * (c.L + 1) * c.n;
    std::vector<uint64_t> wide(relin_key, relin_key + words);
    return hecuda_evk_create(h, wide.data(), out);
}
int32_t hecuda_u32_bfv_relinearize(const hecuda_context *h, const hecuda_evk *evk, const uint32_t *ct3, int32_t l, uint32_t *out,
                                   int64_t batch) {
    int32_t rc = need_word32(h);
    if (rc) return rc;
    Io32Scope scope;
    return hecuda_bfv_relinearize(h, evk, reinterpret_cast<const uint64_t *>(ct3), l, reinterpret_cast<uint64_t *>(out), batch);
}
int32_t hecuda_u32_bfv_mod_switch_down(const hecuda_context *h, const uint32_t *ct, int32_t polys, int32_t l, uint32_t *out,
                                       int64_t batch) {
    int32_t rc = need_word32(h);
    if (rc) return rc;
    Io32Scope scope;
    return hecuda_bfv_mod_switch_down(h, reinterpret_cast<const uint64_t *>(ct), polys, l, reinterpret_cast<uint64_t *>(out), batch);
}
int32_t hecuda_u32_bfv_multiply_relinearize(const hecuda_context *h, const hecuda_evk *evk, const uint32_t *lhs, const uint32_t *rhs,
                                            int32_t mod_switch, uint32_t *out, int64_t batch) {
    int32_t rc = need_word32(h);
    if (rc) return rc;
    Io32Scope scope;
    return hecuda_bfv_multiply_relinearize(h, evk, reinterpret_cast<const uint64_t *>(lhs), reinterpret_cast<const uint64_t *>(rhs),
                                           mod_switch, reinterpret_cast<uint64_t *>(out), batch);
}
int32_t hecuda_u32_bfv_relinearize_mod_switch_down(const hecuda_context *h, const hecuda_evk *evk, const uint32_t *ct3, int32_t l,
                                                   uint32_t *out, int64_t batch) {
    int32_t rc = need_word32(h);
    if (rc) return rc;
    Io32Scope scope;
    return hecuda_bfv_relinearize_mod_switch_down(h, evk, reinterpret_cast<const uint64_t *>(ct3), l,
                                                  reinterpret_cast<uint64_t *>(out), batch);
}
int32_t hecuda_u32_evk_set_galois_key(hecuda_evk *evk, uint32_t element, const uint32_t *key) {
    if (!evk || !key) return fail(HECUDA_ERR_INVALID_ARGUMENT, "null argument");
    int32_t rc = need_word32(evk->owner);
    if (rc) return rc;
    std::vector<uint64_t> wide(key, key + evk->words);
    return hecuda_evk_set_galois_key(evk, element, wide.data());
}
int32_t hecuda_u32_bfv_apply_galois(const hecuda_context *h, const hecuda_evk *evk, const uint32_t *ct, int32_t l, uint32_t element,
                                    uint32_t *out, int64_t batch) {
    int32_t rc = need_word32(h);
    if (rc) return rc;
    Io32Scope scope;
    return hecuda_bfv_apply_galois(h, evk, reinterpret_cast<const uint64_t *>(ct), l, element, reinterpret_cast<uint64_t *>(out), batch);
}
int32_t hecuda_u32_bfv_inner_product(const hecuda_context *h, const uint32_t *lhs, const uint32_t *rhs, uint32_t *out, int64_t pairs,
                                     int64_t groups) {
    int32_t rc = need_word32(h);
    if (rc) return rc;
    Io32Scope scope;
    return hecuda_bfv_inner_product(h, reinterpret_cast<const uint64_t *>(lhs), reinterpret_cast<const uint64_t *>(rhs),
                                    reinterpret_cast<uint64_t *>(out), pairs, groups);
}
int32_t hecuda_u32_rnstool_lift_q_to_qbsk(const hecuda_context *h, const uint32_t *polys, uint32_t *out, int64_t count) {
    int32_t rc = need_word32(h);
    if (rc) return rc;
    Io32Scope scope;
    return hecuda_rnstool_lift_q_to_qbsk(h, reinterpret_cast<const uint64_t *>(polys), reinterpret_cast<uint64_t *>(out), count);
}
int32_t hecuda_u32_rnstool_floor_qbsk_to_q(const hecuda_context *h, const uint32_t *polys, uint32_t *out, int64_t count) {
    int32_t rc = need_word32(h);
    if (rc) return rc;
    Io32Scope scope;
    return hecuda_rnstool_floor_qbsk_to_q(h, reinterpret_cast<const uint64_t *>(polys), reinterpret_cast<uint64_t *>(out), count);
}
int32_t hecuda_u32_bfv_encode_simd(const hecuda_context *h, const uint32_t *values, int32_t value_count, int32_t moduli_count,
                                   uint32_t *out, int64_t count) {
    int32_t rc = need_word32(h);
    if (rc) return rc;
    Io32Scope scope;
    return hecuda_bfv_encode_simd(h, reinterpret_cast<const uint64_t *>(values), value_count, moduli_count,
                                  reinterpret_cast<uint64_t *>(out), count);
}
int32_t hecuda_u32_bfv_decode_simd(const hecuda_context *h, const uint32_t *plaintexts, int32_t moduli_count, uint32_t *values,
                                   int64_t count) {
    int32_t rc = need_word32(h);
    if (rc) return rc;
    Io32Scope scope;
    return hecuda_bfv_decode_simd(h, reinterpret_cast<const uint64_t *>(plaintexts), moduli_count,
                                  reinterpret_cast<uint64_t *>(values), count);
}
int32_t hecuda_u32_bfv_plaintext_translate(const hecuda_context *h, const uint32_t *ct, int32_t poly_count, int32_t moduli_count,
                                           const uint32_t *plaintexts, int64_t plaintext_count, int32_t op, uint32_t *out,
                                           int64_t batch) {
    int32_t rc = need_word32(h);
    if (rc) return rc;
    Io32Scope scope;
    return hecuda_bfv_plaintext_translate(h, reinterpret_cast<const uint64_t *>(ct), poly_count, moduli_count,
                                          reinterpret_cast<const uint64_t *>(plaintexts), plaintext_count, op,
                                          reinterpret_cast<uint64_t *>(out), batch);
}

}
```

swift-homomorphic-encryption_b200/csrc/context.cu:

```cuda
#include "context.hpp"

#include <cuda_runtime.h>

#include <cmath>
#include <cstdlib>
#include <cstring>

#include "hostmath.hpp"
#include "ntt_fast.cuh"

namespace hecuda {
using namespace host;


static void fill_barrett(u64 p, u64 &mu1, u64 &mu_hi, u64 &mu_lo) {
    mu1 = (u64)(((u128)1 << 64) / p);
    u128 mu = (p & (p - 1)) == 0 ? ((u128)1 << (128 - (bit_length(p) - 1))) : (~(u128)0) / p;
    mu_hi = (u64)(mu >> 64);
    mu_lo = (u64)mu;
}

static bool build_slot(HostSlot &hs, u64 p, int64_t n, int logn, u64 t, std::vector<ulonglong2> &tw,
                       std::vector<ulonglong2> &itw, std::string &err) {
    if (!is_prime(p) || (p - 1) % (2 * (u64)n) != 0) {
        err = "invalidNttModulus: " + std::to_string(p) + " is not a prime = 1 mod 2N";
        return false;
    }
    if (p >= (1ull << 62)) {
        err = "invalidModulus: " + std::to_string(p) + " exceeds 2^62 - 1";
        return false;
    }
    ModSlot &d = hs.dev;
    std::memset(&d, 0, sizeof(d));
    d.p = p;
    fill_barrett(p, d.mu1, d.mu_hi, d.mu_lo);
    d.bits = bit_length(p);
    d.s_prod = d.bits - 2;
    d.mu_prod = (u64)(((u128)1 << (d.bits + 62)) / p);
    d.red_shift = d.bits > 12 ? d.bits - 12 : 0;
    d.red_recip = (u32)((((u128)1) << (d.red_shift + 32)) / p);
    const u64 psi = min_primitive_root(2 * (u64)n, p);
    const u64 psi_inv = invmod(psi, p);
    hs.roots.assign(n, 1);
    hs.inv_roots.assign(n, 1);
    u64 pw = 1, ipw = 1;
    for (int64_t i = 0; i < n; ++i) {
        unsigned r = bitrev((unsigned)i, logn);
        hs.roots[r] = pw;
        hs.inv_roots[r] = ipw;
        pw = mulmod(pw, psi, p);
        ipw = mulmod(ipw, psi_inv, p);
    }
    tw.resize(n);
    itw.resize(n);
    for (int64_t i = 0; i < n; ++i) {
        tw[i] = make_ulonglong2(hs.roots[i], shoup_factor(hs.roots[i], p));
        itw[i] = make_ulonglong2(hs.inv_roots[i], shoup_factor(hs.inv_roots[i], p));
    }
    const u64 n_inv = invmod((u64)n % p, p);
    const u64 w1_inv = n > 1 ? hs.inv_roots[1] : 1;
    d.r64 = (u64)(((u128)1 << 64) % p);
    {
        u64 inv = p;
        for (int i = 0; i < 6; ++i) inv *= 2 - p * inv;
        d.ninv = 0 - inv;
    }
    const u64 scalings[3] = {1 % p, mulmod(t % p, d.r64, p), d.r64};
    for (int k = 0; k < 3; ++k) {
        ModSlot::InvScale &sc = d.inv_scale[k];
        sc.c0 = mulmod(n_inv, scalings[k], p);
        sc.c0p = shoup_factor(sc.c0, p);
        sc.c1 = mulmod(sc.c0, w1_inv, p);
        sc.c1p = shoup_factor(sc.c1, p);
    }
    return true;
}

static DivRoundConsts build_divround(const std::vector<u64> &base) {
    DivRoundConsts c;
    std::memset(&c, 0, sizeof(c));
    c.l = (int)base.size();
    c.last = base.back();
    c.half = c.last >> 1;
    for (int i = 0; i + 1 < c.l; ++i) {
        const u64 m = base[i];
        c.m[i] = m;
        c.mu1[i] = (u64)(((u128)1 << 64) / m);
        c.half_mod[i] = c.half % m;
        c.inv_w[i] = invmod(c.last % m, m);
        c.inv_wp[i] = shoup_factor(c.inv_w[i], m);
    }
    return c;
}

Context *Context::create(int64_t n, const u64 *coeff_moduli, int nmod, u64 t, std::string &err, int word_bits) {
    if (word_bits != 64 && word_bits != 32) { err = "invalidEncryptionParameters: word size must be 32 or 64"; return nullptr; }
    for (int i = 0; i < nmod; ++i)
        if (coeff_moduli[i] >> (word_bits - 2)) { err = "invalidModulus: " + std::to_string(coeff_moduli[i]) + " exceeds the maximum of this word size"; return nullptr; }
    if (n < 2 || (n & (n - 1)) || n > (1 << 17)) { err = "invalidDegree: N must be a power of two in [2, 2^17]"; return nullptr; }
    if (n > (1 << fast::kSplitLogN)) { err = "unsupportedHeOperation: polynomial degrees above 2^" + std::to_string(fast::kSplitLogN) + " are not supported by the NTT kernels"; return nullptr; }
    if (nmod < 1) { err = "invalidEncryptionParameters: need at least one coefficient modulus"; return nullptr; }
    if (nmod > kMaxL) { err = "invalidEncryptionParameters: more than " + std::to_string(kMaxL) + " coefficient moduli (EncryptionParameters.swift:148)"; return nullptr; }
    if (t < 2) { err = "invalidEncryptionParameters: plaintext modulus"; return nullptr; }
    for (int i = 0; i < nmod; ++i)
        for (int j = 0; j < i; ++j)
            if (coeff_moduli[i] == coeff_moduli[j]) { err = "coprimeModuli: repeated coefficient modulus"; return nullptr; }

    Context *c = new Context();
    c->n = n;
    c->logn = bit_length((u64)n) - 1;
    c->has_ks = nmod >= 2;
    c->L = c->has_ks ? nmod - 1 : 1;
    c->t = t;
    c->word_bits = word_bits;
    c->mtilde = word_bits == 64 ? (1ull << 32) : (1ull << 16);
    c->gamma = word_bits == 64 ? ((1ull << 62) - 40797) : ((1ull << 30) - 20405);
    const u64 kMTilde = c->mtilde;
    cudaGetDevice(&c->device);
    c->sm_count = 1;
    cudaDeviceGetAttribute(&c->sm_count, cudaDevAttrMultiProcessorCount, c->device);
    const int L = c->L;
    c->q.assign(coeff_moduli, coeff_moduli + L);
    c->q_ks = c->has_ks ? coeff_moduli[L] : 0;
    for (u64 qi : c->q)
        if (t >= qi) { err = "invalidEncryptionParameters: plaintext modulus must be below every coefficient modulus"; delete c; return nullptr; }
    c->bsk = smallest_ntt_primes(word_bits - 3, L + 1, (u64)n);
    if ((int)c->bsk.size() != L + 1) { err = "notEnoughPrimes for Bsk"; delete c; return nullptr; }
    for (u64 b : c->bsk)
        for (int i = 0; i < nmod; ++i)
            if (b == coeff_moduli[i]) { err = "coprimeModuli: coefficient modulus collides with the BEHZ base"; delete c; return nullptr; }

    c->aux = c->bsk;
    {
        const char *env = std::getenv("HECUDA_AUX_BASE");
        const bool want_fast = !(env && std::string(env) == "reference");
        const int widths[2] = {30, 55};
        double log_q = 0;
        for (u64 v : c->q) log_q += std::log2((double)v);
        const double log_n = (double)c->logn, log_t = std::log2((double)t);
        for (int wi = 0; wi < 2 && want_fast && c->aux == c->bsk && word_bits == 64; ++wi) {
            std::vector<u64> cand = widths[wi] == 55 ? smallest_ntt_primes(55, L + 1 + nmod, 1ull << 31)
                                                     : smallest_ntt_primes(widths[wi], L + 1 + nmod, (u64)n);
            std::vector<u64> pick;
            for (u64 v : cand) {
                bool used = false;
                for (int i = 0; i < nmod; ++i) used |= coeff_moduli[i] == v;
                if (!used && (int)pick.size() < L + 1) pick.push_back(v);
            }
            double log_aux = 0, log_aux_l = 0;
            for (size_t j = 0; j < pick.size(); ++j) {
                log_aux += std::log2((double)pick[j]);
                if ((int)j < L) log_aux_l += std::log2((double)pick[j]);
            }
            const bool enough = (int)pick.size() == L + 1 && log_aux >= log_q + log_n + 4 &&
                                log_aux_l + std::log2((double)pick.back()) >= log_t + log_n + log_q + 5;
            if (enough) c->aux = pick;
        }
    }
    c->aux_is_reference = c->aux == c->bsk;

    c->simd = is_prime(t) && (t - 1) % (2 * (u64)n) == 0;
    const int nslots = (c->aux_is_reference ? 2 * L + 2 : 3 * L + 3) + (c->simd ? 1 : 0);
    c->slots.resize(nslots);
    std::vector<u64> slot_mod(nslots);
    if (c->simd) slot_mod[c->slot_t()] = t;
    for (int i = 0; i < L; ++i) slot_mod[c->slot_q(i)] = c->q[i];
    for (int j = 0; j <= L; ++j) slot_mod[c->slot_bsk(j)] = c->bsk[j];
    slot_mod[c->slot_ks()] = c->q_ks;
    if (!c->aux_is_reference)
        for (int j = 0; j <= L; ++j) slot_mod[c->slot_aux(j)] = c->aux[j];
    const size_t table_bytes = sizeof(ulonglong2) * (size_t)n;
    const bool fast = c->logn >= fast::kMinLogN && c->logn <= fast::kMaxLogN;
    const bool split = c->logn == fast::kSplitLogN;
    const int half_logn = c->logn - 1;
    const int64_t half_n = n / 2;
    const int threads = (int)((split ? half_n : n) / 16);
    const size_t tr_bytes = (fast || split) ? sizeof(ulonglong2) * (size_t)15 * threads : 0;
    const size_t half_bytes = sizeof(ulonglong2) * (size_t)half_n;
    const size_t slot_bytes = 2 * table_bytes + (split ? 2 * (2 * half_bytes + 2 * tr_bytes) : 2 * tr_bytes);
    if (cudaMalloc(&c->d_pool, slot_bytes * nslots) != cudaSuccess) { err = "cudaMalloc failed for twiddle tables"; delete c; return nullptr; }
    std::vector<ulonglong2> tw, itw, tr(15 * (size_t)threads), itr(15 * (size_t)threads), twh, itwh;
    std::vector<ModSlot> dev_slots(split ? 3 * nslots : nslots);
    c->split_slot_base = split ? nslots : 0;
    for (int s = 0; s < nslots; ++s) {
        if (s == c->slot_ks() && !c->has_ks) {
            std::memset(&c->slots[s].dev, 0, sizeof(ModSlot));
            dev_slots[s] = c->slots[s].dev;
            continue;
        }
        if (!build_slot(c->slots[s], slot_mod[s], n, c->logn, t, tw, itw, err)) { delete c; return nullptr; }
        char *base = (char *)c->d_pool + slot_bytes * s;
        cudaMemcpy(base, tw.data(), table_bytes, cudaMemcpyHostToDevice);
        cudaMemcpy(base + table_bytes, itw.data(), table_bytes, cudaMemcpyHostToDevice);
        c->slots[s].dev.tw = (const ulonglong2 *)base;
        c->slots[s].dev.itw = (const ulonglong2 *)(base + table_bytes);
        if (fast) {
            for (int k = 0; k < 15; ++k)
                for (int tau = 0; tau < threads; ++tau) {
                    tr[(size_t)k * threads + tau] = tw[fast::fwd_last_source(c->logn, k, tau)];
                    itr[(size_t)k * threads + tau] = itw[fast::inv_first_source(c->logn, k, tau)];
                }
            cudaMemcpy(base + 2 * table_bytes, tr.data(), tr_bytes, cudaMemcpyHostToDevice);
            cudaMemcpy(base + 2 * table_bytes + tr_bytes, itr.data(), tr_bytes, cudaMemcpyHostToDevice);
            c->slots[s].dev.tw_t = (const ulonglong2 *)(base + 2 * table_bytes);
            c->slots[s].dev.itw_t = (const ulonglong2 *)(base + 2 * table_bytes + tr_bytes);
        }
        dev_slots[s] = c->slots[s].dev;
        if (split) {
            for (int hh = 0; hh < 2; ++hh) {
                twh.assign(half_n, tw[0]);
                itwh.assign(half_n, itw[0]);
                for (int64_t i = 1; i < half_n; ++i) {
                    const int sp = bit_length((u64)i) - 1;
                    const int64_t src = ((int64_t)(2 + hh) << sp) + (i - ((int64_t)1 << sp));
                    twh[i] = tw[src];
                    itwh[i] = itw[src];
                }
                for (int k = 0; k < 15; ++k)
                    for (int tau = 0; tau < threads; ++tau) {
                        tr[(size_t)k * threads + tau] = twh[fast::fwd_last_source(half_logn, k, tau)];
                        itr[(size_t)k * threads + tau] = itwh[fast::inv_first_source(half_logn, k, tau)];
                    }
                char *hb = base + 2 * table_bytes + hh * (2 * half_bytes + 2 * tr_bytes);
                cudaMemcpy(hb, twh.data(), half_bytes, cudaMemcpyHostToDevice);
                cudaMemcpy(hb + half_bytes, itwh.data(), half_bytes, cudaMemcpyHostToDevice);
                cudaMemcpy(hb + 2 * half_bytes, tr.data(), tr_bytes, cudaMemcpyHostToDevice);
                cudaMemcpy(hb + 2 * half_bytes + tr_bytes, itr.data(), tr_bytes, cudaMemcpyHostToDevice);
                ModSlot v = c->slots[s].dev;
                v.tw = (const ulonglong2 *)hb;
                v.itw = (const ulonglong2 *)(hb + half_bytes);
                v.tw_t = (const ulonglong2 *)(hb + 2 * half_bytes);
                v.itw_t = (const ulonglong2 *)(hb + 2 * half_bytes + tr_bytes);
                dev_slots[nslots + 2 * s + hh] = v;
            }
        }
    }
    if (cudaMalloc(&c->d_slots, sizeof(ModSlot) * dev_slots.size()) != cudaSuccess) { err = "cudaMalloc failed"; delete c; return nullptr; }
    cudaMemcpy(c->d_slots, dev_slots.data(), sizeof(ModSlot) * dev_slots.size(), cudaMemcpyHostToDevice);

    const u64 *Q = c->q.data();
    auto build_behz = [&](const std::vector<u64> &base, bool reference_base, LiftConsts &lf, FloorConsts &fl) {
    const u64 *BSK = base.data();
    const u64 msk = base[L];
    auto slot_of = [&](int j) { return reference_base ? c->slot_bsk(j) : c->slot_aux(j); };
    std::memset(&lf, 0, sizeof(lf));
    lf.L = L;
    bool h_primes = true;
    for (int j = 0; j <= L; ++j) h_primes &= fast::class_of_modulus(BSK[j], bit_length(BSK[j])) == fast::kNarrowH;
    lf.h_primes = h_primes ? 1 : 0;
    {
        const u64 q_mod_mt = prod_mod(Q, L, kMTilde);
        lf.neg_inv_q_mt = (u32)((kMTilde - invmod(q_mod_mt, kMTilde)) % kMTilde);
    }
    for (int i = 0; i < L; ++i) {
        const u64 qi = Q[i];
        lf.q[i] = qi;
        const u64 inv_punct = invmod(punctured_mod(Q, L, i, qi), qi);
        lf.in_w[i] = mulmod(kMTilde % qi, inv_punct, qi);
        lf.in_wp[i] = shoup_factor(lf.in_w[i], qi);
        lf.punct_mt[i] = (u32)punctured_mod(Q, L, i, kMTilde);
    }
    lf.mt_mask = (u32)(kMTilde - 1);
    lf.mt_half = (u32)(kMTilde >> 1);
    for (int j = 0; j <= L; ++j) lf.neg_off[j] = ((kMTilde + BSK[j] - 1) / BSK[j]) * BSK[j] - kMTilde;
    for (int j = 0; j <= L; ++j) {
        const u64 bj = BSK[j];
        lf.b[j] = bj;
        lf.b_ninv[j] = c->slots[slot_of(j)].dev.ninv;
        const u64 r64 = c->slots[slot_of(j)].dev.r64;
        const u64 mt_inv = mulmod(invmod(kMTilde % bj, bj), r64, bj);
        for (int i = 0; i < L; ++i) lf.mat[j][i] = mulmod(punctured_mod(Q, L, i, bj), mt_inv, bj);
        lf.qr[j] = mulmod(prod_mod(Q, L, bj), mt_inv, bj);
    }
    std::memset(&fl, 0, sizeof(fl));
    fl.L = L;
    fl.h_primes = lf.h_primes;
    const u64 b_mod_msk = prod_mod(BSK, L, msk);
    const u64 r64_msk = c->slots[slot_of(L)].dev.r64;
    const u64 b_inv_msk = mulmod(invmod(b_mod_msk, msk), r64_msk, msk);
    fl.a_msk = (msk - b_inv_msk) % msk;
    for (int i = 0; i < L; ++i) {
        const u64 qi = Q[i];
        fl.q[i] = qi;
        fl.q_ninv[i] = c->slots[c->slot_q(i)].dev.ninv;
        fl.q_mu1[i] = c->slots[c->slot_q(i)].dev.mu1;
        const u64 r64 = c->slots[c->slot_q(i)].dev.r64;
        fl.inq_w[i] = invmod(punctured_mod(Q, L, i, qi), qi);
        fl.inq_wp[i] = shoup_factor(fl.inq_w[i], qi);
        for (int k = 0; k < L; ++k) fl.omat[i][k] = mulmod(punctured_mod(BSK, L, k, qi), r64, qi);
        fl.b_mod_q[i] = mulmod(prod_mod(BSK, L, qi), r64, qi);
        fl.neg_b_mod_q[i] = (qi - fl.b_mod_q[i]) % qi;
    }
    for (int j = 0; j <= L; ++j) {
        const u64 bj = BSK[j];
        fl.b[j] = bj;
        fl.b_ninv[j] = c->slots[slot_of(j)].dev.ninv;
        const u64 q_inv = mulmod(invmod(prod_mod(Q, L, bj), bj), c->slots[slot_of(j)].dev.r64, bj);
        fl.fq[j] = q_inv;
        for (int i = 0; i < L; ++i) {
            const u64 v = mulmod(punctured_mod(Q, L, i, bj), q_inv, bj);
            fl.fmat[j][i] = (bj - v) % bj;
        }
    }
    for (int k = 0; k < L; ++k) {
        const u64 bk = BSK[k];
        fl.inb_w[k] = invmod(punctured_mod(BSK, L, k, bk), bk);
        fl.inb_wp[k] = shoup_factor(fl.inb_w[k], bk);
        fl.amat[k] = mulmod(punctured_mod(BSK, L, k, msk), b_inv_msk, msk);
    }
    };
    build_behz(c->bsk, true, c->lift, c->floor);
    if (c->aux_is_reference) {
        c->lift_mul = c->lift;
        c->floor_mul = c->floor;
    } else {
        build_behz(c->aux, false, c->lift_mul, c->floor_mul);
    }

    auto check_ranges = [&](const std::vector<u64> &base, LiftConsts &lf, FloorConsts &fl) -> bool {
        u64 qmax = 0, bmax = 0;
        for (u64 v : c->q) qmax = v > qmax ? v : qmax;
        for (u64 v : base) bmax = v > bmax ? v : bmax;
        const double worst = std::log2((double)(L + 2)) + std::log2((double)qmax) + std::log2((double)bmax);
        if (worst >= 127.0) return false;
        const bool wide = (u128)bmax + (u128)L * qmax >= ((u128)1 << 64);
        lf.wide_sums = fl.wide_sums = wide ? 1 : 0;
        for (int j = 0; j <= L; ++j) lf.b_mu1[j] = (u64)(((u128)1 << 64) / base[j]);
        fl.msk_mu1 = (u64)(((u128)1 << 64) / base[L]);
        return true;
    };
    if (!check_ranges(c->bsk, c->lift, c->floor) || !check_ranges(c->aux, c->lift_mul, c->floor_mul)) {
        err = "unsupportedHeOperation: " + std::to_string(L) + " ciphertext moduli of this size overflow the 128-bit lazy sums";
        delete c;
        return nullptr;
    }

    {
        u64 mmax = c->q_ks;
        for (u64 v : c->q) mmax = v > mmax ? v : mmax;
        if (std::log2((double)L) + 2 * std::log2((double)mmax) >= 128.0) {
            err = "unsupportedHeOperation: " + std::to_string(L) + " moduli of this size overflow the key-switching accumulator";
            delete c;
            return nullptr;
        }
    }

    c->translate.resize(L + 1);
    for (int l = 1; l <= L; ++l) {
        TranslateConsts &tc = c->translate[l];
        std::memset(&tc, 0, sizeof(tc));
        tc.l = l;
        tc.t = t;
        tc.t_threshold = (t + 1) / 2;
        tc.q_mod_t = prod_mod(Q, l, t);
        tc.q_mod_t_p = shoup_factor(tc.q_mod_t, t);
        for (int i = 0; i < l; ++i) {
            const u64 qi = Q[i];
            tc.q[i] = qi;
            tc.delta[i] = mulmod((qi - tc.q_mod_t % qi) % qi, invmod(t % qi, qi), qi);
            tc.delta_p[i] = shoup_factor(tc.delta[i], qi);
        }
    }

    if (c->simd) {
        std::vector<int32_t> matrix(n), inverse(n);
        const u64 mask = 2 * (u64)n - 1;
        u64 g = 1;
        for (int64_t i = 0; i < n / 2; ++i) {
            matrix[i] = (int32_t)bitrev((unsigned)((g - 1) >> 1), c->logn);
            matrix[n / 2 + i] = (int32_t)bitrev((unsigned)((mask - g) >> 1), c->logn);
            g = (g * 3) & mask;
        }
        for (int64_t i = 0; i < n; ++i) inverse[matrix[i]] = (int32_t)i;
        if (cudaMalloc(&c->d_simd_matrix, sizeof(int32_t) * 2 * (size_t)n) != cudaSuccess) { err = "cudaMalloc failed"; delete c; return nullptr; }
        c->d_simd_inverse = c->d_simd_matrix + n;
        cudaMemcpy(c->d_simd_matrix, matrix.data(), sizeof(int32_t) * (size_t)n, cudaMemcpyHostToDevice);
        cudaMemcpy(c->d_simd_inverse, inverse.data(), sizeof(int32_t) * (size_t)n, cudaMemcpyHostToDevice);
    }

    c->ks_divround.resize(L + 1);
    c->ms_divround.resize(L + 1);
    for (int l = 1; l <= L; ++l) {
        std::vector<u64> base(c->q.begin(), c->q.begin() + l);
        if (l >= 2) c->ms_divround[l] = build_divround(base);
        if (!c->has_ks) continue;
        base.push_back(c->q_ks);
        c->ks_divround[l] = build_divround(base);
    }
    cudaError_t e = cudaDeviceSynchronize();
    if (e != cudaSuccess) { err = std::string("CUDA error during context setup: ") + cudaGetErrorString(e); delete c; return nullptr; }
    return c;
}

Context::~Context() {
    if (d_pool) cudaFree(d_pool);
    if (d_slots) cudaFree(d_slots);
    if (d_simd_matrix) cudaFree(d_simd_matrix);
}

NttRowMap Context::map_q(int rows) const {
    NttRowMap m;
    std::memset(&m, 0, sizeof(m));
    m.rows_per_poly = rows;
    m.group = 1;
    m.src_mod = 0;
    m.src_poly_stride = 0;
    for (int r = 0; r < rows; ++r) m.slot[r] = (unsigned char)slot_q(r);
    return m;
}
NttRowMap Context::map_qbsk() const {
    NttRowMap m;
    std::memset(&m, 0, sizeof(m));
    m.rows_per_poly = 2 * L + 1;
    m.group = 1;
    m.src_mod = 0;
    m.src_poly_stride = 0;
    for (int r = 0; r < L; ++r) m.slot[r] = (unsigned char)slot_q(r);
    for (int j = 0; j <= L; ++j) m.slot[L + j] = (unsigned char)slot_bsk(j);
    return m;
}
NttRowMap Context::map_qaux() const {
    NttRowMap m = map_qbsk();
    if (!aux_is_reference)
        for (int j = 0; j <= L; ++j) m.slot[L + j] = (unsigned char)slot_aux(j);
    return m;
}
NttRowMap Context::map_ks(int l) const {
    NttRowMap m;
    std::memset(&m, 0, sizeof(m));
    m.rows_per_poly = l + 1;
    m.group = 1;
    m.src_mod = 0;
    m.src_poly_stride = 0;
    for (int r = 0; r < l; ++r) m.slot[r] = (unsigned char)slot_q(r);
    m.slot[l] = (unsigned char)slot_ks();
    return m;
}
NttRowMap Context::map_single(int slot) const {
    NttRowMap m;
    std::memset(&m, 0, sizeof(m));
    m.rows_per_poly = 1;
    m.group = 1;
    m.src_mod = 0;
    m.src_poly_stride = 0;
    m.slot[0] = (unsigned char)slot;
    return m;
}
NttRowMap Context::map_ks_digits(int l, long long target_poly_stride) const {
    NttRowMap m = map_ks(l);
    m.rows_per_poly = (l + 1) * l;
    m.group = l;
    m.src_mod = l;
    m.src_poly_stride = target_poly_stride;
    for (int j = 0; j < l; ++j) m.src_slot[j] = (unsigned char)slot_q(j);
    return m;
}
int Context::find_slot(u64 modulus) const {
    for (size_t s = 0; s < slots.size(); ++s)
        if (slots[s].dev.p == modulus) return (int)s;
    return -1;
}

}
```

swift-homomorphic-encryption_b200/csrc/context.hpp:

```cpp
#pragma once
#include <cstdint>
#include <string>
#include <vector>

#include "modarith.cuh"

namespace hecuda {

constexpr int kMaxL = 32;
constexpr int kMaxSlots = 3 * kMaxL + 4;
constexpr int kMaxRows = 2 * kMaxL + 1;

struct ModSlot {
    u64 p;
    u64 mu1;
    u64 mu_hi, mu_lo;
    u64 mu_prod;
    int s_prod;
    int bits;
    int red_shift;
    u32 red_recip;
    u64 ninv;
    u64 r64;
    struct InvScale { u64 c0, c0p, c1, c1p; } inv_scale[3];
    const ulonglong2 *tw;
    const ulonglong2 *itw;
    const ulonglong2 *tw_t;
    const ulonglong2 *itw_t;
};

enum { kScalePlain = 0, kScaleTMont = 1, kScaleMont = 2 };

struct NttRowMap {
    int rows_per_poly;
    int group;
    unsigned char slot[kMaxRows + 1];
    int src_mod;
    long long src_poly_stride;
    unsigned char src_slot[kMaxRows + 1];
};

struct LiftConsts {
    int L;
    int wide_sums;
    u64 b_mu1[kMaxL + 1];
    u64 q[kMaxL];
    u64 in_w[kMaxL], in_wp[kMaxL];
    u32 punct_mt[kMaxL];
    u32 neg_inv_q_mt;
    u32 mt_mask, mt_half;
    u64 neg_off[kMaxL + 1];
    u64 b[kMaxL + 1], b_ninv[kMaxL + 1];
    u64 mat[kMaxL + 1][kMaxL];
    u64 qr[kMaxL + 1];
    int h_primes;
};

struct FloorConsts {
    int L;
    int wide_sums;
    u64 msk_mu1;
    u64 q[kMaxL], q_ninv[kMaxL], q_mu1[kMaxL];
    u64 inq_w[kMaxL], inq_wp[kMaxL];
    u64 b[kMaxL + 1], b_ninv[kMaxL + 1];
    u64 fq[kMaxL + 1];
    u64 fmat[kMaxL + 1][kMaxL];
    u64 inb_w[kMaxL], inb_wp[kMaxL];
    u64 amat[kMaxL];
    u64 a_msk;
    u64 omat[kMaxL][kMaxL];
    u64 b_mod_q[kMaxL], neg_b_mod_q[kMaxL];
    int h_primes;
};

struct DivRoundConsts {
    int l;
    u64 m[kMaxL + 1], mu1[kMaxL + 1];
    u64 last, half;
    u64 half_mod[kMaxL + 1];
    u64 inv_w[kMaxL + 1], inv_wp[kMaxL + 1];
};

struct TranslateConsts {
    int l;
    u64 t, t_threshold;
    u64 q_mod_t, q_mod_t_p;
    u64 q[kMaxL];
    u64 delta[kMaxL], delta_p[kMaxL];
};

struct HostSlot {
    ModSlot dev;
    std::vector<u64> roots, inv_roots;
};

class Context {
   public:
    static Context *create(int64_t n, const u64 *coeff_moduli, int nmod, u64 t, std::string &err, int word_bits = 64);
    ~Context();

    int64_t n;
    int logn;
    int word_bits = 64;
    u64 mtilde = 1ull << 32;
    u64 gamma = (1ull << 62) - 40797;
    int L;
    u64 t;
    int device;
    int sm_count;
    std::vector<u64> q;
    u64 q_ks;
    bool has_ks = true;
    std::vector<u64> bsk;
    std::vector<u64> aux;
    bool aux_is_reference = true;
    std::vector<HostSlot> slots;
    ModSlot *d_slots = nullptr;
    int split_slot_base = 0;
    LiftConsts lift;
    FloorConsts floor;
    LiftConsts lift_mul;
    FloorConsts floor_mul;
    std::vector<DivRoundConsts> ks_divround;
    std::vector<DivRoundConsts> ms_divround;
    void *d_pool = nullptr;
    bool simd = false;
    int32_t *d_simd_matrix = nullptr;
    int32_t *d_simd_inverse = nullptr;
    std::vector<TranslateConsts> translate;

    int slot_q(int i) const { return i; }
    int slot_bsk(int j) const { return L + j; }
    int slot_ks() const { return 2 * L + 1; }
    int slot_aux(int j) const { return aux_is_reference ? slot_bsk(j) : 2 * L + 2 + j; }
    int slot_t() const { return simd ? (aux_is_reference ? 2 * L + 2 : 3 * L + 3) : -1; }
    NttRowMap map_q(int rows) const;
    NttRowMap map_qbsk() const;
    NttRowMap map_qaux() const;
    NttRowMap map_ks(int l) const;
    NttRowMap map_single(int slot) const;
    NttRowMap map_ks_digits(int l, long long target_poly_stride) const;
    int find_slot(u64 modulus) const;
};

}
```

swift-homomorphic-encryption_b200/csrc/kernels.cuh:

```cuda
#pragma once
#include <cuda_runtime.h>

#include <atomic>
#include <string>

#include "context.hpp"

namespace hecuda {

extern std::atomic<unsigned long long> g_kernel_launches;

cudaError_t launch_ntt_forward(const Context &ctx, const NttRowMap &map, const u64 *in, u64 *out, int64_t rows,
                               cudaStream_t stream);
cudaError_t launch_ntt_inverse(const Context &ctx, const NttRowMap &map, const u64 *in, u64 *out, int64_t rows,
                               int scale_mode, cudaStream_t stream);

cudaError_t launch_ntt_forward_simple(const Context &ctx, const NttRowMap &map, const u64 *in, u64 *out, int64_t rows,
                                      cudaStream_t stream);
cudaError_t launch_ntt_inverse_simple(const Context &ctx, const NttRowMap &map, const u64 *in, u64 *out, int64_t rows,
                                      int scale_mode, cudaStream_t stream);

bool ntt_fast_supported(const Context &ctx);
cudaError_t launch_ntt_forward_fast(const Context &ctx, const NttRowMap &map, const u64 *in, u64 *out, int64_t rows,
                                    cudaStream_t stream);
cudaError_t launch_ntt_inverse_fast(const Context &ctx, const NttRowMap &map, const u64 *in, u64 *out, int64_t rows,
                                    int scale_mode, cudaStream_t stream);
bool ntt_forward_tensor_supported(const Context &ctx);
cudaError_t launch_ntt_forward_tensor(const Context &ctx, const NttRowMap &map, const u64 *lhs, const u64 *rhs,
                                      const u64 *ext, u64 *ten, int64_t items, cudaStream_t stream);

cudaError_t launch_lift(const Context &ctx, const u64 *in, int polys_in, u64 *ext, int ext_polys, int out_poly_offset,
                        int64_t items, cudaStream_t stream, bool reference_base = false, bool q_rows = true);
cudaError_t launch_tensor(const Context &ctx, const u64 *ext, u64 *ten, int64_t items, cudaStream_t stream,
                          bool reference_base = false);
cudaError_t launch_tensor_sum(const Context &ctx, const u64 *ext, u64 *ten, int64_t pairs, int64_t groups,
                              cudaStream_t stream, bool reference_base = false);
cudaError_t launch_floor(const Context &ctx, const u64 *in, u64 *out, int64_t polys, cudaStream_t stream,
                         bool reference_base = false);

cudaError_t launch_ks_mac(const Context &ctx, const u64 *dig, const u64 *key, int l, u64 *prod, int64_t items,
                          cudaStream_t stream);
cudaError_t launch_ks_finish(const Context &ctx, const u64 *prod, const u64 *base, int64_t base_item_stride, int base_mask,
                             int l, u64 *out, int64_t items, cudaStream_t stream);
cudaError_t launch_galois_coeff(const Context &ctx, const NttRowMap &map, unsigned element, const u64 *in,
                                int64_t in_poly_stride, u64 *out, int64_t out_poly_stride, int64_t polys,
                                cudaStream_t stream);
cudaError_t launch_multiply_power_of_x(const Context &ctx, const NttRowMap &map, long long power, const u64 *in, u64 *out,
                                       int64_t polys, cudaStream_t stream);
cudaError_t launch_galois_eval(const Context &ctx, int rows, unsigned element, const u64 *in, u64 *out, int64_t polys,
                               cudaStream_t stream);

cudaError_t launch_inner_product_plain(const Context &ctx, const u64 *cts, int npoly, int l, int64_t terms, const u64 *pts,
                                       const unsigned char *present, u64 *out, int64_t out_count, cudaStream_t stream);
bool inner_product_plain_small_supported(const Context &ctx, int l);
cudaError_t launch_inner_product_plain_small(const Context &ctx, const u64 *cts, int npoly, int l, int64_t terms, const u32 *pts,
                                             const unsigned char *present, u64 *out, int64_t out_count, cudaStream_t stream);
cudaError_t launch_plaintext_to_eval(const Context &ctx, const u64 *plain, int l, u64 *out, int64_t count,
                                     cudaStream_t stream);

size_t simd_scratch_words(const Context &ctx, bool encode, int l);
cudaError_t launch_encode_simd(const Context &ctx, const u64 *values, int value_count, int l, u64 *out, u64 *scratch,
                               int64_t count, cudaStream_t stream);
cudaError_t launch_decode_simd(const Context &ctx, const u64 *plain, int l, u64 *values, u64 *scratch, int64_t count,
                               cudaStream_t stream);
cudaError_t launch_plaintext_translate(const Context &ctx, const u64 *ct, int polys, int l, const u64 *pt, bool broadcast,
                                       int op, u64 *out, int64_t batch, cudaStream_t stream);

struct CodecConsts {
    int rows;
    int width[kMaxRows];
    long long byte_offset[kMaxRows + 1];
};
bool codec_consts(const Context &ctx, const NttRowMap &map, int skip, CodecConsts &c, std::string &err);
long long serialized_poly_bytes(const CodecConsts &c);
cudaError_t launch_poly_load(const Context &ctx, const CodecConsts &c, int skip, const unsigned char *bytes, u64 *out,
                             int64_t polys, cudaStream_t stream);
cudaError_t launch_poly_serialize(const Context &ctx, const CodecConsts &c, int skip, const u64 *in, unsigned char *bytes,
                                  int64_t polys, cudaStream_t stream);

cudaError_t launch_widen(const u32 *in, u64 *out, int64_t words, cudaStream_t stream);
cudaError_t launch_narrow(const u64 *in, u32 *out, int64_t words, cudaStream_t stream);

cudaError_t launch_mod_switch(const Context &ctx, const u64 *in, int l, u64 *out, int64_t polys, cudaStream_t stream);

}
```

Baseline: 140,400.

## Fold BEHZ floor input scalings into NTT constants and fuse lhs/rhs lift

```diff
diff --git a/swift-homomorphic-encryption_b200/csrc/behz.cu b/swift-homomorphic-encryption_b200/csrc/behz.cu
--- a/swift-homomorphic-encryption_b200/csrc/behz.cu
+++ b/swift-homomorphic-encryption_b200/csrc/behz.cu
@@ -1,19 +1,9 @@
-#include <cstdlib>
-
 #include "kernels.cuh"
 #include "ntt_fast.cuh"
 
 namespace hecuda {
 
 constexpr int kThreads = 128;
-
-static int cols_per_thread() {
-    static const int v = [] {
-        const char *e = std::getenv("HECUDA_BEHZ_COLS");
-        return (e && e[0] == '1') ? 1 : 2;
-    }();
-    return v;
-}
 
 template <int COLS>
 struct Cols {
@@ -22,10 +12,13 @@
 template <int COLS>
 __device__ __forceinline__ Cols<COLS> ldc(const u64 *p) {
     Cols<COLS> r;
-    if (COLS == 2) {
-        const ulonglong2 t = *reinterpret_cast<const ulonglong2 *>(p);
-        r.v[0] = t.x;
-        r.v[COLS - 1] = t.y;
+    if (COLS % 2 == 0) {
+#pragma unroll
+        for (int h = 0; h < COLS / 2; ++h) {
+            const ulonglong2 t = reinterpret_cast<const ulonglong2 *>(p)[h];
+            r.v[2 * h] = t.x;
+            r.v[2 * h + (COLS > 1)] = t.y;
+        }
     } else {
         r.v[0] = *p;
     }
@@ -33,56 +26,88 @@
 }
 template <int COLS>
 __device__ __forceinline__ void stc(u64 *p, const u64 (&v)[COLS]) {
-    if (COLS == 2) *reinterpret_cast<ulonglong2 *>(p) = make_ulonglong2(v[0], v[COLS - 1]);
-    else *p = v[0];
-}
-
-template <int L, int COLS, bool H>
-__global__ void __launch_bounds__(kThreads) lift_kernel(const u64 *__restrict__ in, int polys_in, u64 *__restrict__ ext,
-                                                       int ext_polys, int out_poly_offset,
-                                                       const __grid_constant__ LiftConsts c, int n, bool q_rows) {
-    const int rows_out = q_rows ? 2 * L + 1 : L + 1, aux0 = q_rows ? L : 0;
-    const int coeff = (blockIdx.x * kThreads + threadIdx.x) * COLS;
-    if (coeff >= n) return;
-    const int64_t poly = (int64_t)blockIdx.z * gridDim.y + blockIdx.y;
-    const int64_t item = polys_in == 2 ? (poly >> 1) : poly / polys_in;
-    const int pin = (int)(poly - item * polys_in);
-    const u64 *src = in + poly * L * n + coeff;
-    u64 *dst = ext + ((item * ext_polys + out_poly_offset + pin) * rows_out) * n + coeff;
-    u64 z[COLS][L];
-    u32 acc_mt[COLS];
-#pragma unroll
-    for (int k = 0; k < COLS; ++k) acc_mt[k] = 0;
-#pragma unroll
-    for (int i = 0; i < L; ++i) {
-        const Cols<COLS> x = ldc<COLS>(src + (int64_t)i * n);
-        if (q_rows) stc<COLS>(dst + (int64_t)i * n, x.v);
+    if (COLS % 2 == 0) {
+#pragma unroll
+        for (int h = 0; h < COLS / 2; ++h)
+            reinterpret_cast<ulonglong2 *>(p)[h] = make_ulonglong2(v[2 * h], v[2 * h + (COLS > 1)]);
+    } else {
+        *p = v[0];
+    }
+}
+
+template <int L>
+struct BehzCols {
+    static constexpr int value = L <= 8 ? 2 : 1;
+};
+
+struct ColTiles {
+    long long count;
+    int shift;
+};
+
+template <int COLS>
+__device__ __forceinline__ int tile_col(long long t, const ColTiles &tl) {
+    return (int)(t & ((1ll << tl.shift) - 1)) * (kThreads * COLS) + (int)threadIdx.x * COLS;
+}
+
+template <int ROWS, int COLS>
+__device__ __forceinline__ void load_rows(Cols<COLS> (&x)[ROWS], const u64 *src, int64_t n) {
+#pragma unroll
+    for (int i = 0; i < ROWS; ++i) x[i] = ldc<COLS>(src + (int64_t)i * n);
+}
+
+template <int L, bool H, bool Q_ROWS>
+__global__ void __launch_bounds__(kThreads) lift_kernel(const u64 *__restrict__ lhs, const u64 *__restrict__ rhs,
+                                                       int pin_shift, u64 *__restrict__ ext,
+                                                       const __grid_constant__ LiftConsts c, int n, ColTiles tiles) {
+    constexpr int COLS = BehzCols<L>::value, ROWS_OUT = Q_ROWS ? 2 * L + 1 : L + 1, AUX0 = Q_ROWS ? L : 0;
+    if ((int)threadIdx.x * COLS >= n) return;
+    const int op_shift = rhs ? 1 : 0;
+    auto src_of = [&](long long t) {
+        const int64_t g = t >> tiles.shift, item = g >> (pin_shift + op_shift);
+        const int64_t pin = g & ((1 << pin_shift) - 1);
+        const u64 *base = (op_shift && ((g >> pin_shift) & 1)) ? rhs : lhs;
+        return base + ((item << pin_shift) + pin) * L * n + tile_col<COLS>(t, tiles);
+    };
+    const long long t = blockIdx.x;
+    {
+        Cols<COLS> x[L];
+        load_rows<L, COLS>(x, src_of(t), n);
+        u64 *dst = ext + (t >> tiles.shift) * ROWS_OUT * n + tile_col<COLS>(t, tiles);
+        u64 z[COLS][L];
+        u32 acc_mt[COLS];
+#pragma unroll
+        for (int k = 0; k < COLS; ++k) acc_mt[k] = 0;
+#pragma unroll
+        for (int i = 0; i < L; ++i) {
+            if (Q_ROWS) stc<COLS>(dst + (int64_t)i * n, x[i].v);
+#pragma unroll
+            for (int k = 0; k < COLS; ++k) {
+                z[k][i] = shoup_mul(x[i].v[k], c.in_w[i], c.in_wp[i], c.q[i]);
+                acc_mt[k] += (u32)z[k][i] * c.punct_mt[i];
+            }
+        }
+        u32 r[COLS];
+        bool neg[COLS];
 #pragma unroll
         for (int k = 0; k < COLS; ++k) {
-            z[k][i] = shoup_mul(x.v[k], c.in_w[i], c.in_wp[i], c.q[i]);
-            acc_mt[k] += (u32)z[k][i] * c.punct_mt[i];
-        }
-    }
-    u32 r[COLS];
-    bool neg[COLS];
-#pragma unroll
-    for (int k = 0; k < COLS; ++k) {
-        r[k] = (acc_mt[k] * c.neg_inv_q_mt) & c.mt_mask;
-        neg[k] = r[k] >= c.mt_half;
-    }
-#pragma unroll
-    for (int j = 0; j <= L; ++j) {
-        u64 o[COLS];
-#pragma unroll
-        for (int k = 0; k < COLS; ++k) {
-            const u64 rc = neg[k] ? (u64)r[k] + c.neg_off[j] : (u64)r[k];
-            u128 acc = (u128)rc * c.qr[j];
-#pragma unroll
-            for (int i = 0; i < L; ++i) mac128(acc, z[k][i], c.mat[j][i]);
-            const u64 red = mont_reduce_c<H>(acc, c.b[j], c.b_ninv[j]);
-            o[k] = c.wide_sums ? barrett64(red, c.b[j], c.b_mu1[j]) : csub(red, c.b[j]);
-        }
-        stc<COLS>(dst + (int64_t)(aux0 + j) * n, o);
+            r[k] = (acc_mt[k] * c.neg_inv_q_mt) & c.mt_mask;
+            neg[k] = r[k] >= c.mt_half;
+        }
+#pragma unroll
+        for (int j = 0; j <= L; ++j) {
+            u64 o[COLS];
+#pragma unroll
+            for (int k = 0; k < COLS; ++k) {
+                const u64 rc = neg[k] ? (u64)r[k] + c.neg_off[j] : (u64)r[k];
+                u128 acc = (u128)rc * c.qr[j];
+#pragma unroll
+                for (int i = 0; i < L; ++i) mac128(acc, z[k][i], c.mat[j][i]);
+                const u64 red = mont_reduce_c<H>(acc, c.b[j], c.b_ninv[j]);
+                o[k] = c.wide_sums ? barrett64(red, c.b[j], c.b_mu1[j]) : csub(red, c.b[j]);
+            }
+            stc<COLS>(dst + (int64_t)(AUX0 + j) * n, o);
+        }
     }
 }
 
@@ -181,59 +206,57 @@
     stc<2>(o + 2 * ps, o2);
 }
 
-template <int L, int COLS, bool H>
-__global__ void __launch_bounds__(kThreads) floor_kernel(const u64 *__restrict__ in, u64 *__restrict__ out,
-                                                        const __grid_constant__ FloorConsts c, int n) {
-    constexpr int R = 2 * L + 1;
-    const int coeff = (blockIdx.x * kThreads + threadIdx.x) * COLS;
-    if (coeff >= n) return;
-    const int64_t poly = (int64_t)blockIdx.z * gridDim.y + blockIdx.y;
-    const u64 *src = in + poly * R * n + coeff;
-    u64 *dst = out + poly * L * n + coeff;
-    u64 y[COLS][L];
-#pragma unroll
-    for (int i = 0; i < L; ++i) {
-        const Cols<COLS> x = ldc<COLS>(src + (int64_t)i * n);
-#pragma unroll
-        for (int k = 0; k < COLS; ++k) y[k][i] = shoup_mul(x.v[k], c.inq_w[i], c.inq_wp[i], c.q[i]);
-    }
-    u64 f[COLS][L + 1];
-#pragma unroll
-    for (int j = 0; j <= L; ++j) {
-        const Cols<COLS> xb = ldc<COLS>(src + (int64_t)(L + j) * n);
+template <int L, bool H, bool Q_SCALED>
+__global__ void __launch_bounds__(kThreads, L >= 8 ? 1 : 0) floor_kernel(const u64 *__restrict__ in, u64 *__restrict__ out,
+                                                        const __grid_constant__ FloorConsts c, int n, ColTiles tiles) {
+    constexpr int R = 2 * L + 1, COLS = BehzCols<L>::value;
+    if ((int)threadIdx.x * COLS >= n) return;
+    const long long t = blockIdx.x;
+    {
+        Cols<COLS> x[R];
+        load_rows<R, COLS>(x, in + (t >> tiles.shift) * R * n + tile_col<COLS>(t, tiles), n);
+        u64 y[COLS][L];
+#pragma unroll
+        for (int i = 0; i < L; ++i)
+#pragma unroll
+            for (int k = 0; k < COLS; ++k)
+                y[k][i] = Q_SCALED ? x[i].v[k] : shoup_mul(x[i].v[k], c.inq_w[i], c.inq_wp[i], c.q[i]);
+        u64 f[COLS][L + 1];
+#pragma unroll
+        for (int j = 0; j <= L; ++j) {
+#pragma unroll
+            for (int k = 0; k < COLS; ++k) {
+                u128 acc = (u128)x[L + j].v[k] * c.fq[j];
+#pragma unroll
+                for (int i = 0; i < L; ++i) mac128(acc, y[k][i], c.fmat[j][i]);
+                const u64 red = mont_reduce_c<H>(acc, c.b[j], c.b_ninv[j]);
+                f[k][j] = j == L ? red : c.wide_sums ? barrett64(red, c.b[j], c.b_mu1[j]) : csub(red, c.b[j]);
+            }
+        }
+        const u64 msk = c.b[L];
+        u64 outv[L][COLS];
 #pragma unroll
         for (int k = 0; k < COLS; ++k) {
-            u128 acc = (u128)xb.v[k] * c.fq[j];
-#pragma unroll
-            for (int i = 0; i < L; ++i) mac128(acc, y[k][i], c.fmat[j][i]);
-            f[k][j] = mont_reduce_c<H>(acc, c.b[j], c.b_ninv[j]);
-        }
-    }
-    const u64 msk = c.b[L];
-    u64 outv[L][COLS];
-#pragma unroll
-    for (int k = 0; k < COLS; ++k) {
-        u64 w[L];
-        u128 acc = (u128)f[k][L] * c.a_msk;
-#pragma unroll
-        for (int i = 0; i < L; ++i) {
-            w[i] = shoup_mul(f[k][i], c.inb_w[i], c.inb_wp[i], c.b[i]);
-            mac128(acc, w[i], c.amat[i]);
-        }
-        u64 alpha = mont_reduce_c<H>(acc, msk, c.b_ninv[L]);
-        alpha = c.wide_sums ? barrett64(alpha, msk, c.msk_mu1) : csub(csub(csub(alpha, 4 * msk), 2 * msk), msk);
-        const bool exceeds = alpha > (msk >> 1);
-        const u64 alpha_c = exceeds ? msk - alpha : alpha;
-#pragma unroll
-        for (int i = 0; i < L; ++i) {
-            u128 o = (u128)alpha_c * (exceeds ? c.b_mod_q[i] : c.neg_b_mod_q[i]);
-#pragma unroll
-            for (int kk = 0; kk < L; ++kk) mac128(o, w[kk], c.omat[i][kk]);
-            outv[i][k] = csub(csub(mont_reduce(o, c.q[i], c.q_ninv[i]), 2 * c.q[i]), c.q[i]);
-        }
-    }
-#pragma unroll
-    for (int i = 0; i < L; ++i) stc<COLS>(dst + (int64_t)i * n, outv[i]);
+            const u64 *w = f[k];
+            u128 acc = (u128)f[k][L] * c.a_msk;
+#pragma unroll
+            for (int i = 0; i < L; ++i) mac128(acc, w[i], c.amat[i]);
+            u64 alpha = mont_reduce_c<H>(acc, msk, c.b_ninv[L]);
+            alpha = c.wide_sums ? barrett64(alpha, msk, c.msk_mu1) : csub(csub(csub(alpha, 4 * msk), 2 * msk), msk);
+            const bool exceeds = alpha > (msk >> 1);
+            const u64 alpha_c = exceeds ? msk - alpha : alpha;
+#pragma unroll
+            for (int i = 0; i < L; ++i) {
+                u128 o = (u128)alpha_c * (exceeds ? c.b_mod_q[i] : c.neg_b_mod_q[i]);
+#pragma unroll
+                for (int kk = 0; kk < L; ++kk) mac128(o, w[kk], c.omat[i][kk]);
+                outv[i][k] = csub(csub(mont_reduce(o, c.q[i], c.q_ninv[i]), 2 * c.q[i]), c.q[i]);
+            }
+        }
+        u64 *dst = out + (t >> tiles.shift) * L * n + tile_col<COLS>(t, tiles);
+#pragma unroll
+        for (int i = 0; i < L; ++i) stc<COLS>(dst + (int64_t)i * n, outv[i]);
+    }
 }
 
 __global__ void __launch_bounds__(kThreads) lift_generic_kernel(const u64 *__restrict__ in, int polys_in, u64 *__restrict__ ext,
@@ -274,19 +297,18 @@
     const int64_t poly = (int64_t)blockIdx.z * gridDim.y + blockIdx.y;
     const u64 *src = in + poly * R * n + coeff;
     u64 *dst = out + poly * L * n + coeff;
-    u64 y[kMaxL], f[kMaxL + 1], w[kMaxL];
+    u64 y[kMaxL], f[kMaxL + 1];
     for (int i = 0; i < L; ++i) y[i] = shoup_mul(src[(int64_t)i * n], c.inq_w[i], c.inq_wp[i], c.q[i]);
     for (int j = 0; j <= L; ++j) {
         u128 acc = (u128)src[(int64_t)(L + j) * n] * c.fq[j];
         for (int i = 0; i < L; ++i) mac128(acc, y[i], c.fmat[j][i]);
-        f[j] = mont_reduce(acc, c.b[j], c.b_ninv[j]);
-    }
+        const u64 red = mont_reduce(acc, c.b[j], c.b_ninv[j]);
+        f[j] = j == L ? red : barrett64(red, c.b[j], c.b_mu1[j]);
+    }
+    const u64 *w = f;
     const u64 msk = c.b[L];
     u128 acc = (u128)f[L] * c.a_msk;
-    for (int i = 0; i < L; ++i) {
-        w[i] = shoup_mul(f[i], c.inb_w[i], c.inb_wp[i], c.b[i]);
-        mac128(acc, w[i], c.amat[i]);
-    }
+    for (int i = 0; i < L; ++i) mac128(acc, w[i], c.amat[i]);
     u64 alpha = mont_reduce(acc, msk, c.b_ninv[L]);
     alpha = c.wide_sums ? barrett64(alpha, msk, c.msk_mu1) : csub(csub(csub(alpha, 4 * msk), 2 * msk), msk);
     const bool exceeds = alpha > (msk >> 1);
@@ -319,50 +341,80 @@
         default: return cudaErrorInvalidValue;                                                                        \
     }
 
-template <int COLS, bool H>
-static cudaError_t launch_lift_kernel(int L, dim3 grid, cudaStream_t stream, const u64 *in, int polys_in, u64 *ext,
-                                      int ext_polys, int out_poly_offset, const LiftConsts &consts, int n, bool q_rows) {
-    HE_DISPATCH_L(L, (lift_kernel<LL, COLS, H><<<grid, kThreads, 0, stream>>>(in, polys_in, ext, ext_polys, out_poly_offset,
-                                                                              consts, n, q_rows)));
-    return cudaSuccess;
-}
-template <int COLS, bool H>
-static cudaError_t launch_floor_kernel(int L, dim3 grid, cudaStream_t stream, const u64 *in, u64 *out,
-                                       const FloorConsts &consts, int n) {
-    HE_DISPATCH_L(L, (floor_kernel<LL, COLS, H><<<grid, kThreads, 0, stream>>>(in, out, consts, n)));
-    return cudaSuccess;
-}
-
-static inline dim3 poly_grid(int64_t n, int64_t polys, int cols) {
-    const unsigned gx = (unsigned)((n / cols + kThreads - 1) / kThreads);
+static ColTiles col_tiles(int64_t n, int64_t polys, int cols) {
+    ColTiles tl;
+    tl.shift = 0;
+    while (((int64_t)kThreads * cols << tl.shift) < n) ++tl.shift;
+    tl.count = (long long)polys << tl.shift;
+    return tl;
+}
+
+template <typename... KArgs, typename... Args>
+static cudaError_t launch_tiles(void (*kernel)(KArgs...), const ColTiles &tl, cudaStream_t stream, Args... args) {
+    if (tl.count == 0) return cudaSuccess;
+    if (tl.count > 0x7fffffffLL) return cudaErrorInvalidConfiguration;
+    ++g_kernel_launches;
+    kernel<<<(unsigned)tl.count, kThreads, 0, stream>>>(args..., tl);
+    return cudaGetLastError();
+}
+
+template <bool H, bool Q_ROWS>
+static cudaError_t launch_lift_tiles(const Context &ctx, const u64 *lhs, const u64 *rhs, int pin_shift, u64 *ext,
+                                     int64_t polys_out, const LiftConsts &consts, cudaStream_t stream) {
+    cudaError_t e;
+    HE_DISPATCH_L(ctx.L, (e = launch_tiles(lift_kernel<LL, H, Q_ROWS>, col_tiles(ctx.n, polys_out, BehzCols<LL>::value),
+                                           stream, lhs, rhs, pin_shift, ext, consts, (int)ctx.n)));
+    return e;
+}
+template <bool H, bool Q_SCALED>
+static cudaError_t launch_floor_tiles(const Context &ctx, const u64 *in, u64 *out, int64_t polys,
+                                      const FloorConsts &consts, cudaStream_t stream) {
+    cudaError_t e;
+    HE_DISPATCH_L(ctx.L, (e = launch_tiles(floor_kernel<LL, H, Q_SCALED>, col_tiles(ctx.n, polys, BehzCols<LL>::value),
+                                           stream, in, out, consts, (int)ctx.n)));
+    return e;
+}
+
+static inline dim3 poly_grid(int64_t n, int64_t polys) {
+    const unsigned gx = (unsigned)((n + kThreads - 1) / kThreads);
     const int64_t gy = polys < 32768 ? polys : 32768;
     return dim3(gx ? gx : 1, (unsigned)gy, (unsigned)((polys + gy - 1) / gy));
 }
 
-cudaError_t launch_lift(const Context &ctx, const u64 *in, int polys_in, u64 *ext, int ext_polys, int out_poly_offset,
-                        int64_t items, cudaStream_t stream, bool reference_base, bool q_rows) {
-    const LiftConsts &consts = reference_base ? ctx.lift : ctx.lift_mul;
+static cudaError_t launch_lift_generic(const Context &ctx, const u64 *in, int polys_in, u64 *ext, int ext_polys,
+                                       int out_poly_offset, int64_t items, cudaStream_t stream, const LiftConsts &consts,
+                                       bool q_rows) {
     int64_t polys = items * polys_in;
-    if (polys == 0) return cudaSuccess;
     const int64_t pstride_in = (int64_t)ctx.L * ctx.n;
     while (polys > 0) {
         int64_t slab = polys >= 32768 ? (polys / 32768) * 32768 : polys;
-        const int cols = ctx.L > 16 ? 1 : (ctx.n >= 2 ? cols_per_thread() : 1);
-        const dim3 grid = poly_grid(ctx.n, slab, cols);
         ++g_kernel_launches;
-        if (ctx.L > 16) {
-            lift_generic_kernel<<<grid, kThreads, 0, stream>>>(in, polys_in, ext, ext_polys, out_poly_offset, consts, (int)ctx.n, q_rows);
-        } else {
-            auto launch = cols == 2 ? (consts.h_primes ? launch_lift_kernel<2, true> : launch_lift_kernel<2, false>)
-                                    : (consts.h_primes ? launch_lift_kernel<1, true> : launch_lift_kernel<1, false>);
-            const cudaError_t e = launch(ctx.L, grid, stream, in, polys_in, ext, ext_polys, out_poly_offset, consts, (int)ctx.n, q_rows);
-            if (e != cudaSuccess) return e;
-        }
+        lift_generic_kernel<<<poly_grid(ctx.n, slab), kThreads, 0, stream>>>(in, polys_in, ext, ext_polys, out_poly_offset,
+                                                                              consts, (int)ctx.n, q_rows);
         in += slab * pstride_in;
         ext += (slab / polys_in) * (int64_t)ext_polys * (q_rows ? 2 * ctx.L + 1 : ctx.L + 1) * ctx.n;
         polys -= slab;
     }
     return cudaGetLastError();
+}
+
+cudaError_t launch_lift(const Context &ctx, const u64 *lhs, const u64 *rhs, int polys_in, u64 *ext, int64_t items,
+                        cudaStream_t stream, bool reference_base, bool q_rows) {
+    const LiftConsts &consts = reference_base ? ctx.lift : ctx.lift_mul;
+    if (items == 0) return cudaSuccess;
+    if (polys_in != 1 && polys_in != 2) return cudaErrorInvalidValue;
+    const int ops = rhs ? 2 : 1;
+    if (ctx.L > 16) {
+        cudaError_t e = launch_lift_generic(ctx, lhs, polys_in, ext, ops * polys_in, 0, items, stream, consts, q_rows);
+        if (e == cudaSuccess && rhs)
+            e = launch_lift_generic(ctx, rhs, polys_in, ext, ops * polys_in, polys_in, items, stream, consts, q_rows);
+        return e;
+    }
+    const int64_t polys_out = items * ops * polys_in;
+    const int pin_shift = polys_in == 2 ? 1 : 0;
+    auto launch = consts.h_primes ? (q_rows ? launch_lift_tiles<true, true> : launch_lift_tiles<true, false>)
+                                  : (q_rows ? launch_lift_tiles<false, true> : launch_lift_tiles<false, false>);
+    return launch(ctx, lhs, rhs, pin_shift, ext, polys_out, consts, stream);
 }
 
 cudaError_t launch_tensor(const Context &ctx, const u64 *ext, u64 *ten, int64_t items, cudaStream_t stream,
@@ -376,11 +428,10 @@
         tc.ninv[r] = ctx.slots[map.slot[r]].dev.ninv;
         tc.h[r] = fast::class_of_modulus(tc.p[r], ctx.slots[map.slot[r]].dev.bits) == fast::kNarrowH ? 1 : 0;
     }
-    const int cols = ctx.n >= 2 ? cols_per_thread() : 1;
     bool any_h = false;
     for (int r = 0; r < tc.R; ++r) any_h |= tc.h[r] != 0;
-    auto k = cols == 2 ? (any_h ? tensor_kernel<2, true> : tensor_kernel<2, false>) : (any_h ? tensor_kernel<1, true> : tensor_kernel<1, false>);
-    const unsigned gx = (unsigned)((ctx.n / cols + kThreads - 1) / kThreads);
+    auto k = any_h ? tensor_kernel<2, true> : tensor_kernel<2, false>;
+    const unsigned gx = (unsigned)((ctx.n / 2 + kThreads - 1) / kThreads);
     for (int64_t done = 0; done < items;) {
         const int64_t chunk = (items - done) > 65535 ? 65535 : (items - done);
         dim3 grid(gx ? gx : 1, (unsigned)tc.R, (unsigned)chunk);
@@ -423,24 +474,23 @@
     return cudaGetLastError();
 }
 
+bool floor_takes_scaled_q(const Context &ctx) { return ctx.L <= 16; }
+
 cudaError_t launch_floor(const Context &ctx, const u64 *in, u64 *out, int64_t polys, cudaStream_t stream,
-                         bool reference_base) {
+                         bool reference_base, bool q_scaled) {
     if (polys == 0) return cudaSuccess;
     const FloorConsts &consts = reference_base ? ctx.floor : ctx.floor_mul;
+    if (ctx.L <= 16) {
+        auto launch = consts.h_primes ? (q_scaled ? launch_floor_tiles<true, true> : launch_floor_tiles<true, false>)
+                                      : (q_scaled ? launch_floor_tiles<false, true> : launch_floor_tiles<false, false>);
+        return launch(ctx, in, out, polys, consts, stream);
+    }
+    if (q_scaled) return cudaErrorInvalidValue;
     const int R = 2 * ctx.L + 1;
     while (polys > 0) {
         int64_t slab = polys >= 32768 ? (polys / 32768) * 32768 : polys;
-        const int cols = ctx.L > 16 ? 1 : (ctx.n >= 2 ? cols_per_thread() : 1);
-        const dim3 grid = poly_grid(ctx.n, slab, cols);
         ++g_kernel_launches;
-        if (ctx.L > 16) {
-            floor_generic_kernel<<<grid, kThreads, 0, stream>>>(in, out, consts, (int)ctx.n);
-        } else {
-            auto launch = cols == 2 ? (consts.h_primes ? launch_floor_kernel<2, true> : launch_floor_kernel<2, false>)
-                                    : (consts.h_primes ? launch_floor_kernel<1, true> : launch_floor_kernel<1, false>);
-            const cudaError_t e = launch(ctx.L, grid, stream, in, out, consts, (int)ctx.n);
-            if (e != cudaSuccess) return e;
-        }
+        floor_generic_kernel<<<poly_grid(ctx.n, slab), kThreads, 0, stream>>>(in, out, consts, (int)ctx.n);
         in += slab * (int64_t)R * ctx.n;
         out += slab * (int64_t)ctx.L * ctx.n;
         polys -= slab;
diff --git a/swift-homomorphic-encryption_b200/csrc/capi.cu b/swift-homomorphic-encryption_b200/csrc/capi.cu
--- a/swift-homomorphic-encryption_b200/csrc/capi.cu
+++ b/swift-homomorphic-encryption_b200/csrc/capi.cu
@@ -113,19 +113,19 @@
     cudaError_t e;
     u64 *ext = scratch, *ten = scratch + 4 * poly_words * items;
     const NttRowMap map = c.map_qaux();
+    const bool scaled = floor_takes_scaled_q(c);
+    const int inv_scale = scaled ? kScaleTMontFloor : kScaleTMont;
     if (ntt_forward_tensor_supported(c)) {
-        if ((e = launch_lift(c, lhs, 2, ext, 4, 0, items, s, false, false)) != cudaSuccess) return e;
-        if ((e = launch_lift(c, rhs, 2, ext, 4, 2, items, s, false, false)) != cudaSuccess) return e;
+        if ((e = launch_lift(c, lhs, rhs, 2, ext, items, s, false, false)) != cudaSuccess) return e;
         if ((e = launch_ntt_forward_tensor(c, map, lhs, rhs, ext, ten, items, s)) != cudaSuccess) return e;
-        if ((e = launch_ntt_inverse(c, map, ten, ten, items * 3 * R, kScaleTMont, s)) != cudaSuccess) return e;
-        return launch_floor(c, ten, out, items * 3, s);
-    }
-    if ((e = launch_lift(c, lhs, 2, ext, 4, 0, items, s)) != cudaSuccess) return e;
-    if ((e = launch_lift(c, rhs, 2, ext, 4, 2, items, s)) != cudaSuccess) return e;
+        if ((e = launch_ntt_inverse(c, map, ten, ten, items * 3 * R, inv_scale, s)) != cudaSuccess) return e;
+        return launch_floor(c, ten, out, items * 3, s, false, scaled);
+    }
+    if ((e = launch_lift(c, lhs, rhs, 2, ext, items, s)) != cudaSuccess) return e;
     if ((e = launch_ntt_forward(c, map, ext, ext, items * 4 * R, s)) != cudaSuccess) return e;
     if ((e = launch_tensor(c, ext, ten, items, s)) != cudaSuccess) return e;
-    if ((e = launch_ntt_inverse(c, map, ten, ten, items * 3 * R, kScaleTMont, s)) != cudaSuccess) return e;
-    return launch_floor(c, ten, out, items * 3, s);
+    if ((e = launch_ntt_inverse(c, map, ten, ten, items * 3 * R, inv_scale, s)) != cudaSuccess) return e;
+    return launch_floor(c, ten, out, items * 3, s, false, scaled);
 }
 
 cudaError_t keyswitch_chunk(const Context &c, u64 *scratch, const u64 *key, const u64 *target, int64_t target_stride,
@@ -168,12 +168,13 @@
     u64 *ext = scratch, *ten = scratch + 4 * poly_words * items;
     const NttRowMap map = c.map_qaux();
     cudaError_t e;
-    if ((e = launch_lift(c, lhs, 2, ext, 4, 0, items, s)) != cudaSuccess) return e;
-    if ((e = launch_lift(c, rhs, 2, ext, 4, 2, items, s)) != cudaSuccess) return e;
+    const bool scaled = floor_takes_scaled_q(c);
+    if ((e = launch_lift(c, lhs, rhs, 2, ext, items, s)) != cudaSuccess) return e;
     if ((e = launch_ntt_forward(c, map, ext, ext, items * 4 * R, s)) != cudaSuccess) return e;
     if ((e = launch_tensor_sum(c, ext, ten, pairs, groups, s)) != cudaSuccess) return e;
-    if ((e = launch_ntt_inverse(c, map, ten, ten, groups * 3 * R, kScaleTMont, s)) != cudaSuccess) return e;
-    return launch_floor(c, ten, out, groups * 3, s);
+    if ((e = launch_ntt_inverse(c, map, ten, ten, groups * 3 * R, scaled ? kScaleTMontFloor : kScaleTMont, s)) != cudaSuccess)
+        return e;
+    return launch_floor(c, ten, out, groups * 3, s, false, scaled);
 }
 size_t inner_product_scratch_words(const Context &c, int64_t pairs) {
     return (size_t)(4 * pairs + 3) * (2 * c.L + 1) * c.n;
@@ -519,7 +520,7 @@
     std::vector<HostIo> in = {{(const u64 *)polys, in_words}};
     return host_pipeline(h, count, std::max<int64_t>(1, (int64_t)((size_t)4 * 1024 * 1024 / out_words)), 0, in, (u64 *)out, out_words,
                          [&](Workspace &w, const std::vector<const u64 *> &d_in, u64 *d_out, int64_t n_items) {
-                             return launch_lift(c, d_in[0], 1, d_out, 1, 0, n_items, w.stream, true);
+                             return launch_lift(c, d_in[0], nullptr, 1, d_out, n_items, w.stream, true);
                          });
 }
 int32_t hecuda_rnstool_floor_qbsk_to_q(const hecuda_context *h, const uint64_t *polys, uint64_t *out, int64_t count) {
diff --git a/swift-homomorphic-encryption_b200/csrc/context.cu b/swift-homomorphic-encryption_b200/csrc/context.cu
--- a/swift-homomorphic-encryption_b200/csrc/context.cu
+++ b/swift-homomorphic-encryption_b200/csrc/context.cu
@@ -20,7 +20,7 @@
     mu_lo = (u64)mu;
 }
 
-static bool build_slot(HostSlot &hs, u64 p, int64_t n, int logn, u64 t, std::vector<ulonglong2> &tw,
+static bool build_slot(HostSlot &hs, u64 p, int64_t n, int logn, u64 t, u64 floor_w, std::vector<ulonglong2> &tw,
                        std::vector<ulonglong2> &itw, std::string &err) {
     if (!is_prime(p) || (p - 1) % (2 * (u64)n) != 0) {
         err = "invalidNttModulus: " + std::to_string(p) + " is not a prime = 1 mod 2N";
@@ -65,8 +65,8 @@
         for (int i = 0; i < 6; ++i) inv *= 2 - p * inv;
         d.ninv = 0 - inv;
     }
-    const u64 scalings[3] = {1 % p, mulmod(t % p, d.r64, p), d.r64};
-    for (int k = 0; k < 3; ++k) {
+    const u64 scalings[4] = {1 % p, mulmod(t % p, d.r64, p), d.r64, mulmod(mulmod(t % p, d.r64, p), floor_w % p, p)};
+    for (int k = 0; k < 4; ++k) {
         ModSlot::InvScale &sc = d.inv_scale[k];
         sc.c0 = mulmod(n_inv, scalings[k], p);
         sc.c0p = shoup_factor(sc.c0, p);
@@ -188,7 +188,8 @@
             dev_slots[s] = c->slots[s].dev;
             continue;
         }
-        if (!build_slot(c->slots[s], slot_mod[s], n, c->logn, t, tw, itw, err)) { delete c; return nullptr; }
+        const u64 floor_w = s < L ? invmod(punctured_mod(c->q.data(), L, s, slot_mod[s]), slot_mod[s]) : 1;
+        if (!build_slot(c->slots[s], slot_mod[s], n, c->logn, t, floor_w, tw, itw, err)) { delete c; return nullptr; }
         char *base = (char *)c->d_pool + slot_bytes * s;
         cudaMemcpy(base, tw.data(), table_bytes, cudaMemcpyHostToDevice);
         cudaMemcpy(base + table_bytes, itw.data(), table_bytes, cudaMemcpyHostToDevice);
@@ -295,19 +296,16 @@
         const u64 bj = BSK[j];
         fl.b[j] = bj;
         fl.b_ninv[j] = c->slots[slot_of(j)].dev.ninv;
-        const u64 q_inv = mulmod(invmod(prod_mod(Q, L, bj), bj), c->slots[slot_of(j)].dev.r64, bj);
+        fl.b_mu1[j] = (u64)(((u128)1 << 64) / bj);
+        u64 q_inv = mulmod(invmod(prod_mod(Q, L, bj), bj), c->slots[slot_of(j)].dev.r64, bj);
+        if (j < L) q_inv = mulmod(q_inv, invmod(punctured_mod(BSK, L, j, bj), bj), bj);
         fl.fq[j] = q_inv;
         for (int i = 0; i < L; ++i) {
             const u64 v = mulmod(punctured_mod(Q, L, i, bj), q_inv, bj);
             fl.fmat[j][i] = (bj - v) % bj;
         }
     }
-    for (int k = 0; k < L; ++k) {
-        const u64 bk = BSK[k];
-        fl.inb_w[k] = invmod(punctured_mod(BSK, L, k, bk), bk);
-        fl.inb_wp[k] = shoup_factor(fl.inb_w[k], bk);
-        fl.amat[k] = mulmod(punctured_mod(BSK, L, k, msk), b_inv_msk, msk);
-    }
+    for (int k = 0; k < L; ++k) fl.amat[k] = mulmod(punctured_mod(BSK, L, k, msk), b_inv_msk, msk);
     };
     build_behz(c->bsk, true, c->lift, c->floor);
     if (c->aux_is_reference) {
diff --git a/swift-homomorphic-encryption_b200/csrc/context.hpp b/swift-homomorphic-encryption_b200/csrc/context.hpp
--- a/swift-homomorphic-encryption_b200/csrc/context.hpp
+++ b/swift-homomorphic-encryption_b200/csrc/context.hpp
@@ -22,14 +22,14 @@
     u32 red_recip;
     u64 ninv;
     u64 r64;
-    struct InvScale { u64 c0, c0p, c1, c1p; } inv_scale[3];
+    struct InvScale { u64 c0, c0p, c1, c1p; } inv_scale[4];
     const ulonglong2 *tw;
     const ulonglong2 *itw;
     const ulonglong2 *tw_t;
     const ulonglong2 *itw_t;
 };
 
-enum { kScalePlain = 0, kScaleTMont = 1, kScaleMont = 2 };
+enum { kScalePlain = 0, kScaleTMont = 1, kScaleMont = 2, kScaleTMontFloor = 3 };
 
 struct NttRowMap {
     int rows_per_poly;
@@ -63,9 +63,9 @@
     u64 q[kMaxL], q_ninv[kMaxL], q_mu1[kMaxL];
     u64 inq_w[kMaxL], inq_wp[kMaxL];
     u64 b[kMaxL + 1], b_ninv[kMaxL + 1];
+    u64 b_mu1[kMaxL + 1];
     u64 fq[kMaxL + 1];
     u64 fmat[kMaxL + 1][kMaxL];
-    u64 inb_w[kMaxL], inb_wp[kMaxL];
     u64 amat[kMaxL];
     u64 a_msk;
     u64 omat[kMaxL][kMaxL];
diff --git a/swift-homomorphic-encryption_b200/csrc/kernels.cuh b/swift-homomorphic-encryption_b200/csrc/kernels.cuh
--- a/swift-homomorphic-encryption_b200/csrc/kernels.cuh
+++ b/swift-homomorphic-encryption_b200/csrc/kernels.cuh
@@ -29,14 +29,15 @@
 cudaError_t launch_ntt_forward_tensor(const Context &ctx, const NttRowMap &map, const u64 *lhs, const u64 *rhs,
                                       const u64 *ext, u64 *ten, int64_t items, cudaStream_t stream);
 
-cudaError_t launch_lift(const Context &ctx, const u64 *in, int polys_in, u64 *ext, int ext_polys, int out_poly_offset,
-                        int64_t items, cudaStream_t stream, bool reference_base = false, bool q_rows = true);
+cudaError_t launch_lift(const Context &ctx, const u64 *lhs, const u64 *rhs, int polys_in, u64 *ext, int64_t items,
+                        cudaStream_t stream, bool reference_base = false, bool q_rows = true);
 cudaError_t launch_tensor(const Context &ctx, const u64 *ext, u64 *ten, int64_t items, cudaStream_t stream,
                           bool reference_base = false);
 cudaError_t launch_tensor_sum(const Context &ctx, const u64 *ext, u64 *ten, int64_t pairs, int64_t groups,
                               cudaStream_t stream, bool reference_base = false);
+bool floor_takes_scaled_q(const Context &ctx);
 cudaError_t launch_floor(const Context &ctx, const u64 *in, u64 *out, int64_t polys, cudaStream_t stream,
-                         bool reference_base = false);
+                         bool reference_base = false, bool q_scaled = false);
 
 cudaError_t launch_ks_mac(const Context &ctx, const u64 *dig, const u64 *key, int l, u64 *prod, int64_t items,
                           cudaStream_t stream);
```

Result: faster. 146,900 (median of 6 runs) (+4.6%).
